# cindytsai/multigrid_poisson_solver

Hardware: AMD Instinct MI355X
Metric: vcycle_mlups (higher is better)
Workload: dtype f64; 1 GPU; V(3,3)-cycle N=8192^2 fp64, 11 levels to N=8, red-black GS(1e-7) coarse solve, cycle-file driver (eager, stream smoother: temporally blocked wave-streaming kernels on the large levels, register-tile kernels on the levels 65..1024, one-workgroup LDS kernel below; halos recomputed, neighbours via DPP lane shifts); N=8192, levels=11

## Files before the change

multigrid_poisson_solver_amd/csrc/mg_cycle.cpp:

```cpp
#include <chrono>
#include <cmath>
#include <cstdarg>
#include <cstdlib>
#include <cstring>
#include <algorithm>
#include <fstream>
#include <map>
#include <sstream>
#include <string>
#include <vector>

#include "mg_internal.h"

namespace mg {
namespace {

struct LevelNode {
    int N = 0;
    double *U = nullptr, *F = nullptr, *D = nullptr;
    LevelNode *nextNode = nullptr, *prevNode = nullptr;
    int step = 0;
    double smoothingError = 0.0;
    int pending_pre = 0;
    int descents = 0;
};

class LevelList {
public:
    explicit LevelList(Pool *pool, size_t elem_bytes = sizeof(double)) : pool_(pool), elem_bytes_(elem_bytes) {}
    ~LevelList() { clear(); }
    void clear()
    {
        while (lastNode_) Remove_back();
        init_ = 1;
    }
    void Push_back(int n)
    {
        LevelNode *nd = new LevelNode;
        const size_t bytes = (size_t)n * n * elem_bytes_;
        nd->N = n;
        nd->U = (double *)pool_->get(bytes);
        nd->F = (double *)pool_->get(bytes);
        nd->D = (double *)pool_->get(bytes);
        if (!firstNode_) {
            firstNode_ = lastNode_ = nd;
            return;
        }
        nd->prevNode = lastNode_;
        lastNode_->nextNode = nd;
        lastNode_ = nd;
    }
    void Remove_back()
    {
        LevelNode *nd = lastNode_;
        if (!nd) return;
        pool_->put(nd->U);
        pool_->put(nd->F);
        pool_->put(nd->D);
        if (firstNode_ == lastNode_) {
            firstNode_ = lastNode_ = nullptr;
        } else {
            lastNode_ = nd->prevNode;
            lastNode_->nextNode = nullptr;
            if (firstNode_ == lastNode_) init_ = 0;
        }
        delete nd;
    }
    LevelNode *last() { return lastNode_; }
    LevelNode *first() { return firstNode_; }
    int depth() const
    {
        int d = 0;
        for (LevelNode *p = firstNode_; p; p = p->nextNode) ++d;
        return d;
    }
    int Get_N() const { return lastNode_->N; }
    int Get_prev_N() const { return lastNode_->prevNode->N; }
    int Get_init() const { return init_; }
    void Set_init(int r) { init_ = r; }
    bool Is_firstNode() const { return firstNode_ == lastNode_ && firstNode_ != nullptr; }

private:
    Pool *pool_;
    size_t elem_bytes_;
    LevelNode *firstNode_ = nullptr, *lastNode_ = nullptr;
    int init_ = 1;
};

struct Text {
    std::string s;
    void printf(const char *fmt, ...)
    {
        char tmp[256];
        va_list ap;
        va_start(ap, fmt);
        vsnprintf(tmp, sizeof tmp, fmt, ap);
        va_end(ap);
        s += tmp;
    }
};

struct ReportItem {
    std::string text;
    int record = -1;
};

}
}

using namespace mg;

struct mg_cycle_plan {
    int flags = 0;
    std::string path;
    double L = 1.0, min_x = 0.0, min_y = 0.0;
    int con_step = 0, con_N = 0, N_max = 0, N_min = 0;
    std::vector<int> sizes;
    std::vector<double> tokens;
    Pool pool;
    LevelList *levels = nullptr;
    double *F_finest = nullptr;
    double *F64 = nullptr, *U64 = nullptr;
    int refinements = 1;
    int refine_it = 0;
    float *F32_res = nullptr;
    bool F32_stale = false;
    double *refine_err_dev = nullptr;
    std::vector<double> refine_err;
    double *err_dev = nullptr;
    size_t err_cap = 0;
    std::vector<mg_node_record> records;
    std::vector<ReportItem> report_items;
    std::string report;
    double *final_U = nullptr;
    int final_N = 0;
    hipGraph_t graph = nullptr;
    hipGraphExec_t graph_exec = nullptr;
    bool graph_ready = false, graph_failed = false;
    int warm_runs = 0;
    hipEvent_t ev_start = nullptr, ev_end[2] = {nullptr, nullptr};
    int end_at = 0;
    bool have_end = false;
    hipStream_t end_stream = nullptr;
    hipEvent_t mark0 = nullptr, mark1 = nullptr;
    NormSink norms;
    std::vector<Context::PendingNorm> graph_norms;
    int last_status = 0;
    bool last_replayed = false;
    std::vector<NodeOp> ops;
    std::vector<k::TailArgs> tails;
    struct Group {
        int depth = 0, first = 0;
        std::vector<int> members;
        size_t items_at = 0;
        std::vector<double *> errs;
    };
    std::vector<Group> sched;
    void *sched_items = nullptr;
    bool sched_ready = false, sched_tried = false;
    int sched_max_batch = 0;
    int sched_smoother = 0;
    double *sched_U = nullptr;
    int sched_N = 0;
    int *gs_slots = nullptr;
    int last_tail = -1;
};

namespace mg {
k::TailArgsF tail_args_f32(const k::TailArgs &a)
{
    k::TailArgsF f;
    memset(&f, 0, sizeof f);
    f.n_levels = a.n_levels;
    f.n_nodes = a.n_nodes;
    for (int i = 0; i < a.n_nodes; ++i) f.nodes[i] = a.nodes[i];
    for (int l = 0; l < a.n_levels; ++l) {
        f.N[l] = a.N[l];
        f.dx2[l] = (float)a.dx2[l];
        f.inv[l] = (float)a.inv[l];
        f.gs_h2[l] = a.gs_h2[l];
        f.gs_inv[l] = a.gs_inv[l];
        if (l + 1 < a.n_levels) {
            const RestrictTable &rt = restrict_table(a.N[l], a.N[l + 1]);
            const ProlongTable &pt = prolong_table(a.N[l + 1], a.N[l]);
            f.r_lo[l] = rt.lo;
            f.r_w[l] = rt.w_f;
            f.p_orow[l] = pt.owner_row;
            f.p_ocol[l] = pt.owner_col;
            f.p_rhi[l] = pt.row_hi_f;
            f.p_rlo[l] = pt.row_lo_f;
            f.p_chi[l] = pt.col_hi_f;
            f.p_clo[l] = pt.col_lo_f;
            f.c_dx[l] = (float)pt.c_dx;
        }
    }
    f.err_dev = a.err_dev;
    f.gs_state = a.gs_state;
    f.trace = a.trace;
    return f;
}

bool scan_tail(const std::vector<double> &tokens, size_t *tok_io, const std::vector<int> &sizes, int at0, int con_step,
               int top_N, double L, k::TailArgs *out, int *node_level)
{
    static const bool disabled = getenv("MG_NO_TAIL") != nullptr;
    if (disabled || con_step < 1 || top_N > k::TAIL_MAX_N || top_N < 3) return false;
    k::TailArgs &a = *out;
    memset(&a, 0, sizeof a);
    a.N[0] = top_N;
    int depth = 0, max_depth = 0, at = at0, n_nodes = 0;
    size_t tok = *tok_io;
    for (;;) {
        if (tok >= tokens.size()) return false;
        const int node = (int)tokens[tok++];
        if (node == 1 && depth == 0) {
            --tok;
            break;
        }
        if (n_nodes >= k::TAIL_MAX_NODES) return false;
        k::TailNode nd;
        memset(&nd, 0, sizeof nd);
        nd.type = node;
        nd.err_slot = -1;
        if (node == -1) {
            if (at + 1 >= (int)sizes.size() || depth + 1 >= k::TAIL_MAX_LEVELS) return false;
            nd.steps = con_step;
            node_level[n_nodes] = depth;
            ++depth;
            a.N[depth] = sizes[(size_t)++at];
            if (a.N[depth] < 3) return false;
            if (depth > max_depth) max_depth = depth;
        } else if (node == 0) {
            if (tok + 1 >= tokens.size()) return false;
            nd.tol = tokens[tok++];
            if ((int)tokens[tok++] != 1) return false;
            node_level[n_nodes] = depth;
        } else if (node == 1) {
            nd.steps = con_step;
            --depth;
            --at;
            node_level[n_nodes] = depth;
        } else {
            return false;
        }
        a.nodes[n_nodes++] = nd;
    }
    if (n_nodes == 0 || at != at0) return false;
    a.n_nodes = n_nodes;
    a.n_levels = max_depth + 1;
    if (!k::tail_fits(a)) return false;
    for (int l = 0; l < a.n_levels; ++l) {
        const double dx = L / (double)(a.N[l] - 1);
        a.dx2[l] = dx * dx;
        a.inv[l] = 1.0 / a.dx2[l];
        a.gs_h2[l] = a.dx2[l];
        a.gs_inv[l] = a.inv[l];
        if (l + 1 < a.n_levels) {
            const RestrictTable &rt = restrict_table(a.N[l], a.N[l + 1]);
            const ProlongTable &pt = prolong_table(a.N[l + 1], a.N[l]);
            if (!rt.lo || !pt.owner_row) return false;
            a.r_lo[l] = rt.lo;
            a.r_w[l] = rt.w;
            a.p_orow[l] = pt.owner_row;
            a.p_ocol[l] = pt.owner_col;
            a.p_rhi[l] = pt.row_hi;
            a.p_rlo[l] = pt.row_lo;
            a.p_chi[l] = pt.col_hi;
            a.p_clo[l] = pt.col_lo;
            a.c_dx[l] = pt.c_dx;
        }
    }
    *tok_io = tok;
    return true;
}
}

namespace {

const double TRIGGER = 0.01;

struct Exec {
    mg_cycle_plan *p;
    Context &c;
    size_t tok = 0;
    int at = 0;
    int status = 0;
    bool capturing = false;
    bool widened = false;
    bool tracing = false;
    bool untraceable = false;

    bool next(double *v)
    {
        if (tok >= p->tokens.size()) return false;
        *v = p->tokens[tok++];
        return true;
    }
    bool next_int(int *v)
    {
        double d;
        if (!next(&d)) return false;
        *v = (int)d;
        return true;
    }
};

int add_record(mg_cycle_plan *p, int node, int N, int steps)
{
    mg_node_record r{node, N, steps, 0.0};
    p->records.push_back(r);
    return (int)p->records.size() - 1;
}

void report_text(mg_cycle_plan *p, const char *t)
{
    if (!(p->flags & MG_CYCLE_REPORT)) return;
    ReportItem it;
    it.text = t;
    p->report_items.push_back(it);
}
void report_smoothing(mg_cycle_plan *p, int record)
{
    if (!(p->flags & MG_CYCLE_REPORT)) return;
    ReportItem it;
    it.record = record;
    p->report_items.push_back(it);
}

double *error_slot(mg_cycle_plan *p, int record) { return p->err_dev + record; }

int trigger_smoothing(Exec &x, LevelNode *lv)
{
    double slope = TRIGGER + 1.0, before = 0.0;
    lv->step = 0;
    while (slope > TRIGGER) {
        mg_doSmoothing(lv->N, x.p->L, lv->U, lv->F, 1, &lv->smoothingError);
        if (x.c.last_error) return lv->step;
        lv->step += 1;
        if (lv->step == 1) {
            before = lv->smoothingError;
            continue;
        }
        slope = std::fabs(lv->smoothingError - before);
        before = lv->smoothingError;
    }
    return lv->step;
}

int matching_up_step(const Exec &x)
{
    const mg_cycle_plan *p = x.p;
    if (p->con_step > 0) return p->con_step;
    if (p->con_step != 0) return -1;
    int depth = 1;
    for (size_t tok = x.tok; tok < p->tokens.size();) {
        const int node = (int)p->tokens[tok++];
        if (node == 2) break;
        if (node == -1) {
            if (tok >= p->tokens.size()) break;
            const int s = (int)p->tokens[tok++];
            if (p->con_N == 0) ++tok;
            if (s != 0) ++depth;
        } else if (node == 0) {
            tok += 2;
        } else if (node == 1) {
            if (tok >= p->tokens.size()) break;
            const int s = (int)p->tokens[tok++];
            if (--depth == 0) return s;
        }
    }
    return -1;
}

void ensure_U(mg_cycle_plan *p, LevelNode *lv)
{
    if (!lv || lv->pending_pre <= 0) return;
    if (p->flags & MG_CYCLE_MIXED) return;
    mg_smooth_pp(lv->N, p->L, nullptr, lv->U, lv->F, lv->pending_pre, nullptr, nullptr, -1);
    lv->pending_pre = 0;
}

void smooth_level(Exec &x, LevelNode *lv, int step, bool zero_start, bool want_D, int record)
{
    mg_cycle_plan *p = x.p;
    const size_t n = (size_t)lv->N * lv->N;
    if (p->flags & MG_CYCLE_FUSED) {
        if (zero_start) {
            mg_smooth_pp(lv->N, p->L, nullptr, lv->U, lv->F, step, error_slot(p, record), want_D ? lv->D : nullptr, -1);
        } else if (!want_D) {
            mg_smooth_pp(lv->N, p->L, lv->U, lv->D, lv->F, step, error_slot(p, record), nullptr, -1);
            std::swap(lv->U, lv->D);
        } else {
            double *tmp = (double *)p->pool.get(n * sizeof(double));
            mg_smooth_pp(lv->N, p->L, lv->U, tmp, lv->F, step, error_slot(p, record), lv->D, -1);
            std::swap(lv->U, tmp);
            p->pool.put(tmp);
        }
        return;
    }
    if (zero_start) mg_fill_zero(lv->U, n);
    {
        double *tmp = (double *)p->pool.get(n * sizeof(double));
        mg_smooth_pp(lv->N, p->L, lv->U, tmp, lv->F, step, error_slot(p, record), nullptr, +1);
        mg_copy(lv->U, tmp, n);
        p->pool.put(tmp);
    }
    if (want_D) {
        mg_getResidual(lv->N, p->L, lv->U, lv->F, lv->D);
        mg_negate(lv->N, lv->D);
    }
}

bool try_tail(Exec &x)
{
    mg_cycle_plan *p = x.p;
    LevelList &cycle = *p->levels;
    if (p->con_N != 1) return false;
    LevelNode *top = cycle.last();
    static const int batch_tail_n = [] { const char *e = getenv("MG_BATCH_TAIL_N"); return e ? atoi(e) : 32; }();
    if (x.tracing && top->N > batch_tail_n) return false;

    k::TailArgs a;
    int node_level[k::TAIL_MAX_NODES];
    size_t tok = x.tok;
    if (!scan_tail(p->tokens, &tok, p->sizes, x.at, p->con_step, top->N, p->L, &a, node_level)) return false;
    const int n_nodes = a.n_nodes;
    if (p->records.size() + (size_t)n_nodes > p->err_cap) return false;
    const int rec0 = (int)p->records.size();
    const char *down = "             *\n             |\n Restriction |\n             |\n             *\n";
    const char *up = "             *\n             |\nProlongation |\n             |\n             *\n";
    for (int i = 0; i < n_nodes; ++i) {
        k::TailNode &nd = a.nodes[i];
        const int N = a.N[node_level[i]];
        if (nd.type == -1) {
            const int rec = add_record(p, -1, N, nd.steps);
            nd.err_slot = rec - rec0;
            report_smoothing(p, rec);
            report_text(p, down);
        } else if (nd.type == 0) {
            add_record(p, 0, N, 0);
            if (p->flags & MG_CYCLE_REPORT) {
                Text t;
                t.printf("          ~Exact Solver~\n");
                t.printf("Current Grid Size N = %d\n", N);
                t.printf("   Use Exact Solver = GaussSeidel Even / Odd\n");
                t.printf("       Target Error = %.3e\n", nd.tol);
                report_text(p, t.s.c_str());
            }
        } else {
            const int rec = add_record(p, 1, N, nd.steps);
            nd.err_slot = rec - rec0;
            report_text(p, up);
            report_smoothing(p, rec);
        }
    }
    if (p->flags & MG_CYCLE_MIXED) {
        k::TailArgsF f = tail_args_f32(a);
        f.F_top = (const float *)top->F;
        f.U_top = (float *)top->U;
        f.err_dev = p->err_dev + rec0;
        f.gs_state = x.c.gs_state;
        ProfScope ps("coarse_tail_f32", top->N, 0.0);
        k::tail_launch_f32(x.c.stream, f);
        x.tok = tok;
        return true;
    }
    a.F_top = top->F;
    a.U_top = top->U;
    a.err_dev = p->err_dev + rec0;
    a.gs_state = x.c.gs_state;
    if (x.tracing) {
        NodeOp op;
        op.kind = 2;
        op.node.N = top->N;
        op.node.F = top->F;
        op.node.out = top->U;
        op.tail = (int)p->tails.size();
        p->tails.push_back(a);
        p->ops.push_back(op);
        x.tok = tok;
        return true;
    }
    static const bool trace_on = getenv("MG_TAIL_TRACE") != nullptr;
    static int traced = 0;
    long long *trace = nullptr;
    if (trace_on && traced < 3 && !x.capturing) {
        (void)hipMalloc((void **)&trace, (k::TAIL_MAX_NODES + 2 + 24 * 8) * sizeof(long long));
        (void)hipMemset(trace, 0, (k::TAIL_MAX_NODES + 2 + 24 * 8) * sizeof(long long));
        a.trace = trace;
    }
    {
        ProfScope ps("coarse_tail", top->N, 0.0);
        k::tail_launch(x.c.stream, a);
    }
    if (trace) {
        std::vector<long long> t((size_t)a.n_nodes + 2);
        (void)hipStreamSynchronize(x.c.stream);
        (void)hipMemcpy(t.data(), trace, t.size() * sizeof(long long), hipMemcpyDeviceToHost);
        ++traced;
        fprintf(stderr, "[tail trace] staging %.2f us;", (double)(t[1] - t[0]) * 0.01);
        for (int i = 0; i < a.n_nodes; ++i)
            fprintf(stderr, " %d@%d:%.2f", a.nodes[i].type, a.N[node_level[i]], (double)(t[(size_t)i + 2] - t[(size_t)i + 1]) * 0.01);
        fprintf(stderr, " us\n");
#ifdef MG_TAIL_PHASES
        std::vector<long long> ph(24 * 8);
        (void)hipMemcpy(ph.data(), trace + k::TAIL_MAX_NODES + 2, ph.size() * sizeof(long long), hipMemcpyDeviceToHost);
        for (int i = 0; i < a.n_nodes && i < 24; ++i) {
            if (a.nodes[i].type == 0) continue;
            fprintf(stderr, "[tail phases] %2d@%-3d cycles:", a.nodes[i].type, a.N[node_level[i]]);
            for (int k = 1; k < 8 && ph[(size_t)i * 8 + k]; ++k) fprintf(stderr, " %lld", ph[(size_t)i * 8 + k] - ph[(size_t)i * 8 + k - 1]);
            fprintf(stderr, "\n");
        }
#endif
        (void)hipFree(trace);
    }
    x.tok = tok;
    return true;
}

bool uses_trigger(const mg_cycle_plan *p);

void run_nodes(Exec &x)
{
    mg_cycle_plan *p = x.p;
    LevelList &cycle = *p->levels;
    const bool fused = (p->flags & MG_CYCLE_FUSED) != 0;
    const bool mixed = (p->flags & MG_CYCLE_MIXED) != 0;
    x.c.defer_norms = true;
    if (!x.tracing) {
        p->norms.begin_window();
        x.c.norm_sink = &p->norms;
    }
    auto fusable_down = [&](int N, int M, int step) {
        const RestrictTable &rt = restrict_table(N, M);
        return step >= 1 && step <= k::stream_max_steps() && x.c.smoother != SMOOTHER_SIMPLE && k::stream_fusable(N) && rt.lo && rt.fusable;
    };
    auto fusable_up = [&](int Nc, int N, int step) {
        const ProlongTable &pt = prolong_table(Nc, N);
        return step >= 1 && step <= k::stream_max_steps() && x.c.smoother != SMOOTHER_SIMPLE && k::stream_fusable(N) && pt.owner_row && pt.fusable;
    };

    for (;;) {
        int node;
        if (!x.next_int(&node)) break;
        if (node == 2) break;
        if (x.c.last_error) { x.status = 10; break; }
        if (p->records.size() >= p->err_cap) { x.status = 11; break; }

        if (node == -1) {
            int step = 0, next_N = 0;
            if (p->con_step == 0) { if (!x.next_int(&step)) { x.status = 3; break; } }
            else step = p->con_step;
            if (p->con_N == 0) { if (!x.next_int(&next_N)) { x.status = 3; break; } }
            else {
                if (x.at + 1 >= (int)p->sizes.size()) { x.status = 4; break; }
                next_N = p->sizes[++x.at];
            }
            if (step == 0) continue;
            if (next_N < 3) { x.status = 7; break; }
            if (x.tracing && (step < 1 || !fused || mixed)) { x.untraceable = true; break; }

            LevelNode *lv = cycle.last();
            const bool keep = (cycle.Get_init() == 0 && cycle.Is_firstNode());
            int rec;
            if (step == -1) {
                if (x.capturing) { x.status = 8; break; }
                if (!keep) mg_fill_zero(lv->U, (size_t)lv->N * lv->N);
                const int done = trigger_smoothing(x, lv);
                rec = add_record(p, -1, lv->N, done);
                p->records[rec].error = lv->smoothingError;
                mg_upload(error_slot(p, rec), &lv->smoothingError, 1);
                mg_getResidual(lv->N, p->L, lv->U, lv->F, lv->D);
                mg_negate(lv->N, lv->D);
                report_smoothing(p, rec);
                cycle.Push_back(next_N);
                if (!cycle.last()->U || !cycle.last()->F || !cycle.last()->D) { x.status = 14; break; }
                mg_restrict_signed(lv->N, lv->D, next_N, cycle.last()->F, +1);
            } else if (mixed) {
                if (keep) { x.status = 15; break; }
                rec = add_record(p, -1, lv->N, step);
                report_smoothing(p, rec);
                cycle.Push_back(next_N);
                if (!cycle.last()->U || !cycle.last()->F || !cycle.last()->D) { x.status = 14; break; }
                lv->pending_pre = 0;
                if (p->con_step > 0 && recompute_available(next_N, lv->N, step, p->con_step)) {
                    smooth_restrict_f32_no_out(lv->N, p->L, (float *)lv->U, (float *)lv->F, step, error_slot(p, rec), next_N,
                                               (float *)cycle.last()->F);
                    lv->pending_pre = step;
                } else {
                    mg_smooth_restrict_f32(lv->N, p->L, nullptr, (float *)lv->U, (float *)lv->F, step, error_slot(p, rec), next_N,
                                           (float *)cycle.last()->F);
                }
                if (x.c.last_error) { x.status = 15; break; }
                report_text(p, "             *\n             |\n Restriction |\n             |\n             *\n");
                if (!try_tail(x) && next_N <= k::TAIL_MAX_N) { x.status = 15; break; }
                continue;
            } else if (fused) {
                if (x.tracing) {
                    if (keep || !fusable_down(lv->N, next_N, step)) { x.untraceable = true; break; }
                    if (lv->descents > 0) {
                        const size_t bytes = (size_t)lv->N * lv->N * sizeof(double);
                        p->pool.put(lv->U);
                        p->pool.put(lv->D);
                        lv->U = (double *)p->pool.get(bytes);
                        lv->D = (double *)p->pool.get(bytes);
                        lv->pending_pre = 0;
                    }
                }
                lv->descents++;
                rec = add_record(p, -1, lv->N, step);
                report_smoothing(p, rec);
                cycle.Push_back(next_N);
                if (!cycle.last()->U || !cycle.last()->F || !cycle.last()->D || !lv->U || !lv->D) { x.status = 14; break; }
                double *Fc = cycle.last()->F;
                lv->pending_pre = 0;
                const int up_step = keep ? -1 : matching_up_step(x);
                if (up_step > 0 && recompute_available(next_N, lv->N, step, up_step)) {
                    smooth_restrict_no_out(lv->N, p->L, lv->U, lv->F, step, error_slot(p, rec), next_N, Fc);
                    lv->pending_pre = step;
                } else if (!keep) {
                    mg_smooth_restrict(lv->N, p->L, nullptr, lv->U, lv->F, step, error_slot(p, rec), next_N, Fc);
                } else {
                    double *tmp = (double *)p->pool.get((size_t)lv->N * lv->N * sizeof(double));
                    mg_smooth_restrict(lv->N, p->L, lv->U, tmp, lv->F, step, error_slot(p, rec), next_N, Fc);
                    std::swap(lv->U, tmp);
                    p->pool.put(tmp);
                }
                report_text(p, "             *\n             |\n Restriction |\n             |\n             *\n");
                try_tail(x);
                continue;
            } else {
                rec = add_record(p, -1, lv->N, step);
                smooth_level(x, lv, step, !keep, true, rec);
                report_smoothing(p, rec);
                cycle.Push_back(next_N);
                if (!cycle.last()->U || !cycle.last()->F || !cycle.last()->D) { x.status = 14; break; }
                mg_restrict_signed(lv->N, lv->D, next_N, cycle.last()->F, +1);
            }
            report_text(p, "             *\n             |\n Restriction |\n             |\n             *\n");
        } else if (node == 0) {
            double tol;
            int option;
            if (!x.next(&tol) || !x.next_int(&option)) { x.status = 3; break; }
            LevelNode *lv = cycle.last();
            if (x.tracing) { x.untraceable = true; break; }
            if (mixed) { x.status = 15; break; }
            if (x.capturing && lv->N > k::gs_single_workgroup_max_n()) { x.status = 8; break; }
            mg_doExactSolver(lv->N, p->L, lv->U, lv->F, tol, option);
            if (x.c.last_error) { x.status = 5; break; }
            add_record(p, 0, lv->N, 0);
            if (p->flags & MG_CYCLE_REPORT) {
                Text t;
                t.printf("          ~Exact Solver~\n");
                t.printf("Current Grid Size N = %d\n", lv->N);
                if (option == 0) t.printf("   Use Exact Solver = Inverse Matrix\n");
                if (option == 1) t.printf("   Use Exact Solver = GaussSeidel Even / Odd\n");
                t.printf("       Target Error = %.3e\n", tol);
                report_text(p, t.s.c_str());
            }
        } else if (node == 1) {
            int step;
            if (p->con_step == 0) { if (!x.next_int(&step)) { x.status = 3; break; } }
            else step = p->con_step;
            if (p->con_N != 0) x.at--;
            if (cycle.depth() < 2) { x.status = 6; break; }

            LevelNode *coarse = cycle.last();
            LevelNode *fine = coarse->prevNode;
            const char *arrow = "             *\n             |\nProlongation |\n             |\n             *\n";
            if (mixed) {
                if (step <= 0) { x.status = 15; break; }
                const int rec = add_record(p, 1, fine->N, step);
                const bool last_node = fine->N == p->N_max && p->refine_it == 0 && k::stream_fusable(fine->N) &&
                                       prolong_table(coarse->N, fine->N).fusable &&
                                       (x.tok >= p->tokens.size() || (int)p->tokens[x.tok] == 2);
                const int pre = fine->pending_pre;
                if (pre > 0 && !recompute_available(coarse->N, fine->N, pre, step)) { x.status = 15; break; }
                fine->pending_pre = 0;
                if (last_node) {
                    if (pre > 0)
                        prolong_smooth_f32_recompute(coarse->N, (const float *)coarse->U, fine->N, p->L, nullptr, p->U64, (const float *)fine->F,
                                                     pre, step, error_slot(p, rec));
                    else
                        prolong_smooth_f32_wide(coarse->N, (const float *)coarse->U, fine->N, p->L, (const float *)fine->U, p->U64,
                                                (const float *)fine->F, step, error_slot(p, rec));
                    x.widened = true;
                } else if (pre > 0) {
                    prolong_smooth_f32_recompute(coarse->N, (const float *)coarse->U, fine->N, p->L, (float *)fine->U, nullptr,
                                                 (const float *)fine->F, pre, step, error_slot(p, rec));
                } else {
                    mg_prolong_smooth_f32(coarse->N, (const float *)coarse->U, fine->N, p->L, (const float *)fine->U, (float *)fine->D,
                                          (float *)fine->F, step, error_slot(p, rec));
                    std::swap(fine->U, fine->D);
                }
                if (x.c.last_error) { x.status = 15; break; }
                cycle.Remove_back();
                report_text(p, arrow);
                report_smoothing(p, rec);
                continue;
            }
            if (x.tracing && (coarse->pending_pre > 0 || !fused || !fusable_up(coarse->N, fine->N, step) ||
                              (fine->pending_pre > 0 && !recompute_available(coarse->N, fine->N, fine->pending_pre, step)))) {
                x.untraceable = true;
                break;
            }
            ensure_U(p, coarse);
            if (fused && step > 0 && fine->pending_pre > 0 && recompute_available(coarse->N, fine->N, fine->pending_pre, step)) {
                const int rec = add_record(p, 1, fine->N, step);
                prolong_smooth_recompute(coarse->N, coarse->U, fine->N, p->L, fine->U, fine->F, fine->pending_pre, step, error_slot(p, rec));
                fine->pending_pre = 0;
                cycle.Remove_back();
                report_text(p, arrow);
                report_smoothing(p, rec);
                continue;
            }
            ensure_U(p, fine);
            if (fused && step > 0) {
                const int rec = add_record(p, 1, fine->N, step);
                mg_prolong_smooth(coarse->N, coarse->U, fine->N, p->L, fine->U, fine->D, fine->F, step,
                                  error_slot(p, rec));
                std::swap(fine->U, fine->D);
                cycle.Remove_back();
                report_text(p, arrow);
                report_smoothing(p, rec);
                continue;
            }
            if (fused) {
                mg_prolongAdd(coarse->N, coarse->U, fine->N, fine->U, fine->D);
                std::swap(fine->U, fine->D);
                cycle.Remove_back();
            } else {
                const size_t nf = (size_t)fine->N * fine->N;
                double *tempU = (double *)p->pool.get(nf * sizeof(double));
                mg_doProlongation(coarse->N, coarse->U, fine->N, tempU);
                cycle.Remove_back();
                mg_doGridAddition(fine->N, fine->U, tempU);
                p->pool.put(tempU);
            }
            report_text(p, arrow);

            if (step == 0) continue;
            LevelNode *lv = cycle.last();
            int rec;
            if (step == -1) {
                if (x.capturing) { x.status = 8; break; }
                const int done = trigger_smoothing(x, lv);
                rec = add_record(p, 1, lv->N, done);
                p->records[rec].error = lv->smoothingError;
                mg_upload(error_slot(p, rec), &lv->smoothingError, 1);
            } else {
                rec = add_record(p, 1, lv->N, step);
                smooth_level(x, lv, step, false, false, rec);
            }
            report_smoothing(p, rec);
        }
    }
    if (x.status == 0 && cycle.last() && cycle.last()->pending_pre > 0) {
        if (x.tracing) x.untraceable = true;
        else if (mixed) x.status = 15;
        else ensure_U(p, cycle.last());
    }
    x.c.norm_sink = nullptr;
    if (!x.tracing && uses_trigger(p)) p->norms.finish(x.c.stream);
    x.c.defer_norms = false;
}

void reset_levels(mg_cycle_plan *p)
{
    LevelList &cycle = *p->levels;
    while (cycle.depth() > 1) cycle.Remove_back();
    cycle.Set_init(1);
    if (cycle.first()) cycle.first()->descents = 0;
    p->records.clear();
    p->report_items.clear();
}

bool same_shape(const mg_cycle_plan *p, const NodeOp &a, const NodeOp &b)
{
    if (a.kind != b.kind || a.node.N != b.node.N) return false;
    if (a.kind == 2) {
        const k::TailArgs &x = p->tails[(size_t)a.tail], &y = p->tails[(size_t)b.tail];
        if (x.n_levels != y.n_levels || x.n_nodes != y.n_nodes) return false;
        for (int l = 0; l < x.n_levels; ++l)
            if (x.N[l] != y.N[l]) return false;
        for (int i = 0; i < x.n_nodes; ++i) {
            const k::TailNode &m = x.nodes[i], &n = y.nodes[i];
            if (m.type != n.type || m.steps != n.steps || m.err_slot != n.err_slot || m.tol != n.tol) return false;
        }
        return true;
    }
    const k::SmoothNode<double> &x = a.node, &y = b.node;
    return x.steps == y.steps && x.pre == y.pre && x.no_out == y.no_out && x.d_sign == y.d_sign && (x.in == nullptr) == (y.in == nullptr) &&
           (x.coarse == nullptr) == (y.coarse == nullptr) && (x.Fc == nullptr) == (y.Fc == nullptr) && x.Nc == y.Nc && x.M == y.M && a.L == b.L;
}

void drop_schedule(mg_cycle_plan *p)
{
    p->sched.clear();
    p->ops.clear();
    p->tails.clear();
    p->sched_ready = false;
    if (p->sched_items) (void)hipFree(p->sched_items);
    p->sched_items = nullptr;
    if (p->gs_slots) p->pool.put(p->gs_slots);
    p->gs_slots = nullptr;
    p->last_tail = -1;
    p->pool.park(false);
    p->pool.release_parked();
}

void build_schedule(mg_cycle_plan *p)
{
    static const bool on = [] { const char *e = getenv("MG_CYCLE_BATCH"); return !e || atoi(e) != 0; }();
    p->sched_tried = true;
    const bool mixed = (p->flags & MG_CYCLE_MIXED) != 0, fused = (p->flags & MG_CYCLE_FUSED) != 0;
    if (!on || !fused || mixed || p->con_N != 1 || p->con_step < 1 || getenv("MG_NO_TAIL")) return;
    {
        std::vector<int> descents(1, 0);
        bool points = false;
        for (size_t tok = 0; tok < p->tokens.size() && !points;) {
            const int node = (int)p->tokens[tok++];
            if (node == 2) break;
            if (node == -1) {
                if (descents.back() > 0) points = true;
                descents.back()++;
                descents.push_back(0);
            } else if (node == 0) {
                tok += 2;
            } else if (node == 1) {
                if (descents.size() < 2) break;
                descents.pop_back();
            }
        }
        if (!points) return;
    }
    Context &c = ctx();
    reset_levels(p);
    c.active_pool = &p->pool;
    p->pool.park(true);
    c.trace = &p->ops;
    c.trace_failed = false;
    static const int batch_recompute_min = [] { const char *e = getenv("MG_BATCH_RECOMPUTE_MIN_N"); return e ? atoi(e) : 1024; }();
    if (!getenv("MG_RECOMPUTE_MIN_N")) c.recompute_min_override = batch_recompute_min;
    Exec x{p, c};
    x.tracing = true;
    run_nodes(x);
    c.recompute_min_override = 0;
    c.trace = nullptr;
    c.active_pool = nullptr;
    const bool ok = x.status == 0 && !x.untraceable && !c.trace_failed && !c.last_error && !p->ops.empty();
    c.trace_failed = false;
    if (!ok) {
        drop_schedule(p);
        return;
    }
    std::map<const void *, int> wrote, read;
    auto depth_of = [](const std::map<const void *, int> &m, const void *k) {
        const auto it = m.find(k);
        return it == m.end() ? 0 : it->second;
    };
    std::vector<int> depth(p->ops.size(), 0);
    for (size_t i = 0; i < p->ops.size(); ++i) {
        const NodeOp &op = p->ops[i];
        const k::SmoothNode<double> &o = op.node;
        const void *in[3] = {o.F, (op.kind != 2 && o.pre == 0) ? (const void *)o.in : nullptr, o.coarse};
        const void *out[2] = {(op.kind == 2 || !o.no_out) ? (const void *)o.out : nullptr, o.Fc};
        int d = 0;
        for (const void *q : in)
            if (q) d = std::max(d, depth_of(wrote, q));
        for (const void *q : out)
            if (q) d = std::max(d, std::max(depth_of(wrote, q), depth_of(read, q)));
        depth[i] = ++d;
        for (const void *q : in)
            if (q) read[q] = std::max(depth_of(read, q), d);
        for (const void *q : out)
            if (q) wrote[q] = d;
    }
    for (size_t i = 0; i < p->ops.size(); ++i) {
        mg_cycle_plan::Group *g = nullptr;
        for (auto &cand : p->sched)
            if (cand.depth == depth[i] && same_shape(p, p->ops[(size_t)cand.first], p->ops[i])) { g = &cand; break; }
        if (!g) {
            p->sched.emplace_back();
            g = &p->sched.back();
            g->depth = depth[i];
            g->first = (int)i;
        }
        g->members.push_back((int)i);
    }
    std::stable_sort(p->sched.begin(), p->sched.end(), [](const mg_cycle_plan::Group &a, const mg_cycle_plan::Group &b) {
        return a.depth != b.depth ? a.depth < b.depth : a.first < b.first;
    });
    p->sched_max_batch = 0;
    for (const auto &g : p->sched) p->sched_max_batch = std::max(p->sched_max_batch, (int)g.members.size());
    if (p->sched_max_batch < 2) {
        drop_schedule(p);
        return;
    }
    if (!p->tails.empty()) {
        p->gs_slots = (int *)p->pool.get(2 * p->tails.size() * sizeof(int));
        if (!p->gs_slots) { drop_schedule(p); return; }
        for (size_t t = 0; t < p->tails.size(); ++t) p->tails[t].gs_state = p->gs_slots + 2 * t;
    }
    std::vector<char> host;
    for (auto &g : p->sched) {
        g.items_at = host.size();
        for (int m : g.members) {
            const NodeOp &o = p->ops[(size_t)m];
            if (o.kind == 2) {
                const k::TailArgs &a = p->tails[(size_t)o.tail];
                const TailBatchItem it{a.F_top, a.U_top, a.err_dev, a.gs_state};
                host.insert(host.end(), (const char *)&it, (const char *)&it + sizeof it);
                p->last_tail = std::max(p->last_tail, o.tail);
            } else {
                const NodeBatchItem it{o.node.in, o.node.F, o.node.coarse, o.node.out, o.node.Fc};
                host.insert(host.end(), (const char *)&it, (const char *)&it + sizeof it);
                g.errs.push_back(o.node.err);
            }
        }
        while (host.size() % 16) host.push_back(0);
    }
    if (hipMalloc(&p->sched_items, host.size()) != hipSuccess || hipMemcpy(p->sched_items, host.data(), host.size(), hipMemcpyHostToDevice) != hipSuccess) {
        (void)hipGetLastError();
        drop_schedule(p);
        return;
    }
    p->pool.park(false);
    p->sched_U = p->final_U = p->levels->last()->U;
    p->sched_N = p->final_N = p->levels->last()->N;
    p->sched_smoother = (int)c.smoother;
    p->sched_ready = true;
    if (getenv("MG_CYCLE_DEBUG")) {
        fprintf(stderr, "[cycle] batched schedule: %zu nodes in %zu launches (largest batch %d), %.1f MiB of arrays\n", p->ops.size(), p->sched.size(),
                p->sched_max_batch, (double)p->pool.bytes_held() / 1048576.0);
        for (const auto &g : p->sched)
            fprintf(stderr, "   depth %2d  %-44s N=%5d x%zu\n", g.depth, p->ops[(size_t)g.first].kind == 2 ? "coarse_tail" : p->ops[(size_t)g.first].name,
                    p->ops[(size_t)g.first].node.N, g.members.size());
    }
}

void replay_schedule(mg_cycle_plan *p)
{
    Context &c = ctx();
    c.defer_norms = true;
    c.norms_at_window_end = true;
    p->norms.begin_window();
    c.norm_sink = &p->norms;
    for (const auto &g : p->sched) {
        const NodeOp &o = p->ops[(size_t)g.first];
        const int n = (int)g.members.size();
        if (o.kind == 2) {
            ProfScope ps(n > 1 ? "coarse_tail (batch)" : "coarse_tail", o.node.N, 0.0);
            k::tail_launch(c.stream, p->tails[(size_t)o.tail], n, (const TailBatchItem *)((const char *)p->sched_items + g.items_at));
        } else if (n == 1) {
            replay_node(o, nullptr);
        } else {
            NodeBatch b;
            b.n = n;
            b.dev = (const NodeBatchItem *)((const char *)p->sched_items + g.items_at);
            b.err_outs = g.errs.data();
            replay_node(o, &b);
        }
    }
    c.norm_sink = nullptr;
    c.defer_norms = false;
    c.norms_at_window_end = false;
    if (p->last_tail >= 0)
        (void)hipMemcpyAsync(c.gs_state, p->gs_slots + 2 * p->last_tail, 2 * sizeof(int), hipMemcpyDeviceToDevice, c.stream);
}

bool uses_trigger(const mg_cycle_plan *p)
{
    if (p->con_step == -1) return true;
    if (p->con_step != 0) return false;
    for (double t : p->tokens)
        if (t == -1.0) return true;
    return false;
}

}

extern "C" {

mg_cycle_plan *mg_cycle_load(const char *path, int flags)
{
    if (!require_ready("mg_cycle_load")) return nullptr;
    std::ifstream f(path);
    if (!f.is_open()) {
        fail(MG_ERR_CYCLE_FILE, "Cannot open file %s", path);
        return nullptr;
    }
    mg_cycle_plan *p = new mg_cycle_plan;
    p->pool.poison(pool_poison_wanted());
    p->norms.pool = &p->pool;
    p->flags = flags;
    p->path = path;
    if (!(f >> p->L >> p->min_x >> p->min_y >> p->con_step >> p->con_N >> p->N_max >> p->N_min)) {
        fail(MG_ERR_CYCLE_FILE, "%s: malformed cycle structure header", path);
        delete p;
        return nullptr;
    }
    if (p->N_max < 3 || p->N_max > 46340 || (p->con_N != 0 && p->N_min < 1)) {
        fail(MG_ERR_CYCLE_FILE, "%s: unusable grid sizes N_max=%d N_min=%d", path, p->N_max, p->N_min);
        delete p;
        return nullptr;
    }
    std::string tok;
    while (f >> tok) {
        char *end = nullptr;
        const double v = strtod(tok.c_str(), &end);
        if (end == tok.c_str()) break;
        p->tokens.push_back(v);
    }
    if (p->con_N == 1) {
        for (int n = p->N_max; n >= p->N_min && n > 0; n /= 2) p->sizes.push_back(n);
    } else if (p->con_N == 2) {
        for (int n = p->N_max; n >= p->N_min; --n) p->sizes.push_back(n);
    }
    size_t nodes = 0;
    for (double t : p->tokens)
        if (t == -1.0 || t == 1.0 || t == 0.0) ++nodes;
    p->err_cap = nodes + 8;
    p->err_dev = (double *)p->pool.get(p->err_cap * sizeof(double));
    const bool mixed = (flags & MG_CYCLE_MIXED) != 0;
    if (mixed && (!(flags & MG_CYCLE_FUSED) || p->con_N != 1 || p->con_step < 1 || p->con_step > k::stream_max_steps())) {
        fail(MG_ERR_UNSUPPORTED, "%s: the mixed-precision mode needs the fused driver, con_N = 1 and a fixed con_step in 1..%d",
             path, k::stream_max_steps());
        delete p;
        return nullptr;
    }
    p->levels = new LevelList(&p->pool, mixed ? sizeof(float) : sizeof(double));
    p->levels->Push_back(p->N_max);
    LevelNode *top = p->levels->last();
    if (!top->U || !top->F || !top->D || !p->err_dev) {
        mg_cycle_destroy(p);
        return nullptr;
    }
    if (mixed) {
        const size_t n = (size_t)top->N * top->N;
        p->F64 = (double *)p->pool.get(n * sizeof(double));
        p->U64 = (double *)p->pool.get(n * sizeof(double));
        if (!p->F64 || !p->U64) {
            mg_cycle_destroy(p);
            return nullptr;
        }
        mg_getSource(top->N, p->L, p->F64, p->min_x, p->min_y);
        mg_to_f32((float *)top->F, p->F64, n);
    } else {
        mg_getSource(top->N, p->L, top->F, p->min_x, p->min_y);
    }
    p->F_finest = top->F;
    static const bool fenced = [] { const char *e = getenv("MG_WINDOW_EVENT_FENCE"); return e && atoi(e) != 0; }();
    for (hipEvent_t *e : {&p->ev_start, &p->ev_end[0], &p->ev_end[1]}) (void)hipEventCreateWithFlags(e, fenced ? hipEventDefault : hipEventDisableSystemFence);
    mg_sync();
    return p;
}

int mg_cycle_enqueue(mg_cycle_plan *p)
{
    if (!require_ready("mg_cycle_enqueue") || !p) return 1;
    Context &c = ctx();
    hipStream_t s = c.stream;
    int status = 0;
    if (!p->sched_tried) build_schedule(p);
    const bool want_graph = (p->flags & MG_CYCLE_GRAPH) && (p->flags & MG_CYCLE_FUSED) && !(p->flags & MG_CYCLE_MIXED) &&
                            !uses_trigger(p) && !p->graph_failed && (!p->sched_ready || (int)c.smoother == p->sched_smoother);
    c.profile_window++;
    const bool timed = !stream_is_capturing(s);
    p->mark0 = p->mark1 = nullptr;
    if (timed) {
        hipEvent_t prev = (p->have_end && p->end_stream == s) ? p->ev_end[p->end_at] : nullptr;
        const hipError_t q = prev ? hipEventQuery(prev) : hipSuccess;
        if (q != hipSuccess) (void)hipGetLastError();
        if (prev && q == hipErrorNotReady) {
            p->mark0 = prev;
        } else {
            (void)hipEventRecord(p->ev_start, s);
            p->mark0 = p->ev_start;
        }
    }

    p->last_replayed = false;
    if (want_graph && p->graph_ready) {
        if (!MG_HIP(hipGraphLaunch(p->graph_exec, s))) status = 9;
        p->last_replayed = status == 0;
        p->norms.pending = p->graph_norms;
        p->norms.unfinished = true;
    } else {
        const bool mixed = (p->flags & MG_CYCLE_MIXED) != 0;
        const int outer = mixed ? p->refinements : 1;
        const size_t n_top = (size_t)p->N_max * p->N_max;
        if (mixed && p->F32_stale) {
            k::convert_to_f32(s, (float *)p->levels->first()->F, p->F64, n_top);
            p->F32_stale = false;
        }
        const bool use_sched = p->sched_ready && (int)c.smoother == p->sched_smoother;
        if (use_sched) {
            p->final_U = p->sched_U;
            p->final_N = p->sched_N;
            const bool capture_now = want_graph && p->warm_runs >= 1;
            bool capturing = false;
            if (capture_now) {
                if (hipStreamBeginCapture(s, hipStreamCaptureModeThreadLocal) == hipSuccess) capturing = true;
                else { (void)hipGetLastError(); p->graph_failed = true; }
            }
            replay_schedule(p);
            status = c.last_error ? 10 : 0;
            if (capturing) {
                hipGraph_t g = nullptr;
                const hipError_t e = hipStreamEndCapture(s, &g);
                if (e == hipSuccess && status == 0 && hipGraphInstantiate(&p->graph_exec, g, nullptr, nullptr, 0) == hipSuccess) {
                    p->graph = g;
                    p->graph_ready = true;
                    p->graph_norms = p->norms.pending;
                    if (!MG_HIP(hipGraphLaunch(p->graph_exec, s))) status = 9;
                    p->last_replayed = status == 0;
                } else {
                    (void)hipGetLastError();
                    if (g) (void)hipGraphDestroy(g);
                    p->graph_failed = true;
                    replay_schedule(p);
                    status = c.last_error ? 10 : 0;
                }
            }
            p->warm_runs++;
        }
        for (int it = 0; it < outer && status == 0 && !use_sched; ++it) {
        reset_levels(p);
        c.active_pool = &p->pool;
        p->refine_it = it;
        if (it > 0) {
            const double dx = p->L / (double)(p->N_max - 1);
            float *dst = p->F32_res ? p->F32_res : (float *)p->levels->first()->F;
            k::refine_residual(s, p->N_max, 1.0 / (dx * dx), p->U64, p->F64, dst, p->refine_err_dev + (it - 1));
            if (p->F32_res) p->levels->first()->F = (double *)p->F32_res;
            else p->F32_stale = true;
        }
        Exec x{p, c};
        const bool capture_now = want_graph && p->warm_runs >= 1;
        if (capture_now) {
            if (hipStreamBeginCapture(s, hipStreamCaptureModeThreadLocal) == hipSuccess) x.capturing = true;
            else { (void)hipGetLastError(); p->graph_failed = true; }
        }
        static const bool dbg = getenv("MG_CYCLE_DEBUG") != nullptr;
        if (dbg) fprintf(stderr, "[cycle] run_nodes: capturing=%d\n", (int)x.capturing);
        run_nodes(x);
        status = x.status;
        if (dbg) fprintf(stderr, "[cycle] run_nodes done: status %d\n", status);
        if (x.capturing) {
            hipGraph_t g = nullptr;
            const hipError_t e = hipStreamEndCapture(s, &g);
            if (dbg) fprintf(stderr, "[cycle] end capture: %s\n", hipGetErrorString(e));
            if (e == hipSuccess && status == 0 && hipGraphInstantiate(&p->graph_exec, g, nullptr, nullptr, 0) == hipSuccess) {
                if (dbg) fprintf(stderr, "[cycle] instantiated\n");
                p->graph = g;
                p->graph_ready = true;
                p->graph_norms = p->norms.pending;
                if (!MG_HIP(hipGraphLaunch(p->graph_exec, s))) status = 9;
                p->last_replayed = status == 0;
                if (dbg) fprintf(stderr, "[cycle] launched: status %d\n", status);
            } else {
                (void)hipGetLastError();
                if (g) (void)hipGraphDestroy(g);
                p->graph_failed = true;
                if (status == 8) status = 0;
                reset_levels(p);
                Exec y{p, c};
                run_nodes(y);
                status = y.status;
            }
        }
        c.active_pool = nullptr;
        p->warm_runs++;
        p->levels->first()->F = p->F_finest;
        LevelNode *last = p->levels->last();
        p->final_U = last->U;
        p->final_N = last->N;
        if (mixed && status == 0 && last->N == p->N_max) {
            if (x.widened) {  }
            else if (it == 0) k::convert_to_f64(s, p->U64, (const float *)last->U, n_top);
            else k::add_widened(s, p->U64, (const float *)last->U, n_top);
            p->final_U = p->U64;
        } else if (mixed && status == 0) {
            status = 15;
        }
        }
    }
    if (timed) {
        p->end_at ^= 1;
        (void)hipEventRecord(p->ev_end[p->end_at], s);
        p->mark1 = p->ev_end[p->end_at];
        p->have_end = true;
        p->end_stream = s;
    }
    p->last_status = status;
    return status;
}

int mg_cycle_collect(mg_cycle_plan *p, mg_cycle_result *out)
{
    if (!require_ready("mg_cycle_collect") || !p) return 1;
    Context &c = ctx();
    memset(out, 0, sizeof *out);
    p->norms.finish(c.stream);
    mg_sync();
    float dev_ms = 0.f;
    if (p->mark0 && p->mark1 && hipEventElapsedTime(&dev_ms, p->mark0, p->mark1) != hipSuccess) (void)hipGetLastError();

    if (!p->records.empty()) {
        std::vector<double> all(p->records.size());
        mg_download(all.data(), p->err_dev, all.size());
        for (size_t i = 0; i < p->records.size(); ++i)
            if (p->records[i].node != 0) p->records[i].error = all[i];
    }

    p->refine_err.clear();
    if ((p->flags & MG_CYCLE_MIXED) && p->refinements > 1 && p->refine_err_dev) {
        p->refine_err.resize((size_t)p->refinements - 1);
        mg_download(p->refine_err.data(), p->refine_err_dev, p->refine_err.size());
    }

    double mg_error = 0.0;
    if (p->flags & (MG_CYCLE_ERROR | MG_CYCLE_REPORT))
        mg_analyticError(p->final_N, p->L, p->final_U, p->min_x, p->min_y, &mg_error);

    if (p->flags & MG_CYCLE_REPORT) {
        Text t;
        for (const ReportItem &it : p->report_items) {
            if (it.record < 0) {
                t.s += it.text;
                continue;
            }
            const mg_node_record &r = p->records[it.record];
            t.printf("          ~Smoothing~\n");
            t.printf("Current Grid Size N = %d\n", r.N);
            t.printf("    Smoothing Steps = %d\n", r.steps);
            t.printf("              Error = %lf\n", r.error);
        }
        t.printf("\n\n===== Final Result =====\n    Error = %lf\n", mg_error);
        p->report = t.s;
    }

    out->status = p->last_status ? p->last_status : (c.last_error ? 10 : 0);
    out->N = p->final_N;
    out->U_dev = p->final_U;
    out->mg_error = mg_error;
    out->time_ms = 0.0;
    out->device_ms = dev_ms;
    out->n_records = (int)p->records.size();
    out->records = p->records.data();
    out->report = p->report.c_str();
    out->graph_replayed = p->last_replayed ? 1 : 0;
    out->schedule_launches = (p->sched_ready && (int)c.smoother == p->sched_smoother) ? (int)p->sched.size() : 0;
    return out->status;
}

int mg_cycle_execute(mg_cycle_plan *p, mg_cycle_result *out)
{
    if (!require_ready("mg_cycle_execute") || !p) return 1;
    mg_sync();
    const auto t0 = std::chrono::steady_clock::now();
    mg_cycle_enqueue(p);
    mg_sync();
    const auto t1 = std::chrono::steady_clock::now();
    const int status = mg_cycle_collect(p, out);
    out->time_ms = std::chrono::duration<double, std::milli>(t1 - t0).count();
    return status;
}

int mg_cycle_set_refinement(mg_cycle_plan *p, int cycles)
{
    if (!require_ready("mg_cycle_set_refinement") || !p) return 1;
    if (!(p->flags & MG_CYCLE_MIXED) || cycles < 1 || cycles > 64) {
        fail(MG_ERR_ARG, "mg_cycle_set_refinement: needs a MG_CYCLE_MIXED plan and 1..64 cycles (got %d)", cycles);
        return 1;
    }
    if (!p->refine_err_dev) {
        p->refine_err_dev = (double *)p->pool.get(64 * sizeof(double));
        if (!p->refine_err_dev) return 1;
    }
    if (cycles > 1 && !p->F32_res) p->F32_res = (float *)p->pool.get((size_t)p->N_max * p->N_max * sizeof(float));
    p->refinements = cycles;
    return 0;
}

int mg_cycle_refinement_errors(mg_cycle_plan *p, double *out, int cap)
{
    if (!p || !out) return 0;
    int n = 0;
    for (; n < (int)p->refine_err.size() && n < cap; ++n) out[n] = p->refine_err[(size_t)n];
    return n;
}

void mg_cycle_destroy(mg_cycle_plan *p)
{
    if (!p) return;
    if (ctx().ready) (void)hipStreamSynchronize(ctx().stream);
    if (p->graph_exec) (void)hipGraphExecDestroy(p->graph_exec);
    if (p->graph) (void)hipGraphDestroy(p->graph);
    for (hipEvent_t e : {p->ev_start, p->ev_end[0], p->ev_end[1]})
        if (e) (void)hipEventDestroy(e);
    if (p->levels) {
        p->levels->clear();
        delete p->levels;
    }
    drop_schedule(p);
    p->norms.release();
    if (p->err_dev) p->pool.put(p->err_dev);
    if (p->refine_err_dev) p->pool.put(p->refine_err_dev);
    if (p->F32_res) p->pool.put(p->F32_res);
    if (p->F64) p->pool.put(p->F64);
    if (p->U64) p->pool.put(p->U64);
    p->pool.trim();
    delete p;
}

int mg_print2File(int N, const double *U_dev, const char *file_name)
{
    if (!require_ready("mg_print2File")) return 1;
    std::vector<double> U((size_t)N * N);
    mg_download(U.data(), U_dev, U.size());
    FILE *o = fopen(file_name, "w");
    if (!o) {
        fail(MG_ERR_ARG, "Cannot open file %s", file_name);
        return 1;
    }
    for (int j = N - 1; j >= 0; --j)
        for (int i = 0; i < N; ++i) fprintf(o, i == N - 1 ? "%lf\n" : "%lf,", U[i + (size_t)N * j]);
    fclose(o);
    return 0;
}

int mg_cycle_main(int argc, char **argv)
{
    if (argc != 3) {
        printf("[ ERROR ]: Wrong input numbers of parameter.\n");
        return 1;
    }
    printf("OpenMP threads = %d\n", atoi(argv[1]));
    printf("Cycle structure file name = %s\n", argv[2]);
    const char *dev = getenv("MG_DEVICE");
    if (mg_init(dev ? atoi(dev) : 0) != 0) return 1;
    const char *mixed = getenv("MG_MIXED"), *refine = getenv("MG_REFINE");
    const bool want_mixed = (mixed && atoi(mixed) != 0) || (refine && atoi(refine) > 1);
    mg_cycle_plan *plan = mg_cycle_load(argv[2], MG_CYCLE_FUSED | MG_CYCLE_REPORT | MG_CYCLE_ERROR | (want_mixed ? MG_CYCLE_MIXED : 0));
    if (!plan) {
        printf("[ ERROR ]: Cannot open file %s\n", argv[2]);
        return 1;
    }
    if (refine && atoi(refine) > 1 && mg_cycle_set_refinement(plan, atoi(refine)) != 0) {
        printf("[ ERROR ]: %s\n", mg_last_error_string());
        mg_cycle_destroy(plan);
        return 1;
    }
    mg_cycle_result res;
    if (const char *w = getenv("MG_WARMUP"))
        for (int i = 0; i < atoi(w); ++i) mg_cycle_execute(plan, &res);
    const int status = mg_cycle_execute(plan, &res);
    if (status != 0) {
        printf("[ ERROR ]: cycle structure file is malformed (status %d)\n", status);
        mg_cycle_destroy(plan);
        return 1;
    }
    fputs(res.report, stdout);
    printf("Time Used = %lf (ms)\n", res.time_ms);
    std::string name = std::string("Sol_HIP_") + argv[2];
    mg_print2File(res.N, res.U_dev, name.c_str());
    printf("Output file name = %s\n", name.c_str());
    mg_cycle_destroy(plan);
    mg_finalize();
    return 0;
}

}
```

multigrid_poisson_solver_amd/csrc/mg_internal.h:

```cpp
#pragma once

#include <hip/hip_runtime_api.h>

#include <cstddef>
#include <cstdint>
#include <cstdio>
#include <map>
#include <string>
#include <utility>
#include <vector>

#include "mg_hip.h"

namespace mg {

enum ErrorCode {
    MG_OK = 0,
    MG_ERR_HIP = 1,
    MG_ERR_ARG = 2,
    MG_ERR_UNSUPPORTED = 3,
    MG_ERR_NOT_INIT = 4,
    MG_ERR_CYCLE_FILE = 5,
    MG_ERR_COMM = 6,
};

void fail(int code, const char *fmt, ...);
bool hip_ok(hipError_t e, const char *what, const char *file, int line);
#define MG_HIP(expr) ::mg::hip_ok((expr), #expr, __FILE__, __LINE__)

struct RestrictTable {
    int *lo = nullptr;
    double *w = nullptr;
    int *inv = nullptr;
    double *inv_w = nullptr;
    float *w_f = nullptr, *inv_w_f = nullptr;
    bool fusable = false;
};
struct ProlongTable {
    int *owner_row = nullptr, *owner_col = nullptr;
    double *row_hi = nullptr, *row_lo = nullptr;
    double *col_hi = nullptr, *col_lo = nullptr;
    float *row_hi_f = nullptr, *row_lo_f = nullptr, *col_hi_f = nullptr, *col_lo_f = nullptr;
    double c_dx = 0.0;
    bool fusable = false;
    bool fusable4 = false;
    bool closed_form = false;
};
inline const double *weights_as(double, const double *w, const float *) { return w; }
inline const float *weights_as(float, const double *, const float *w_f) { return w_f; }

struct RowWindow {
    int base = 0, rows = 0, own_lo = 0, own_hi = 0;
    int norm_lo = -1, norm_hi = -1;
};

class Pool {
public:
    void *get(size_t bytes);
    void put(void *p);
    void trim();
    size_t bytes_held() const { return held_; }
    void park(bool on) { park_ = on; }
    void release_parked();
    void poison(bool on) { poison_ = on; }
private:
    std::multimap<size_t, void *> free_;
    std::map<void *, size_t> live_;
    std::vector<std::pair<size_t, void *>> parked_;
    bool park_ = false;
    bool poison_ = false;
    size_t held_ = 0;
};
bool pool_poison_wanted();
void poison_block(void *p, size_t bytes);

enum Smoother { SMOOTHER_STREAM = 0, SMOOTHER_SIMPLE = 1, SMOOTHER_STREAM_ONLY = 2 };

struct NodeOp;
struct NormSink;

struct Context {
    bool ready = false;
    int device = -1;
    hipStream_t own_stream = nullptr;
    hipStream_t stream = nullptr;
    int n_cu = 256;
    Pool pool;
    Pool *active_pool = nullptr;
    int recompute_min_override = 0;
    std::vector<NodeOp> *trace = nullptr;
    bool trace_failed = false;
    Smoother smoother = SMOOTHER_STREAM;
    int source_mode = 0;
    int source_identical = -1;
    double *partials = nullptr;
    size_t partials_cap = 0;
    std::vector<void *> retired;
    struct PendingNorm { const double *part; int n; int N; double *out; };
    bool defer_norms = false;
    bool norms_at_window_end = false;
    std::vector<PendingNorm> pending_norms;
    double *norm_arena = nullptr;
    size_t norm_arena_cap = 0, norm_arena_used = 0;
    size_t norm_window_total = 0;
    NormSink *norm_sink = nullptr;
    double *scalars = nullptr;
    int *gs_state = nullptr;
    double *host_scalars = nullptr;
    int *host_ints = nullptr;
    std::map<std::pair<int, int>, RestrictTable> rtab;
    std::map<std::pair<int, int>, ProlongTable> ptab;
    int last_error = 0;
    std::string last_error_text;
    bool abort_on_error = true;
    bool profiling = false;
    int profile_min_N = 0;
    int profile_every = 1;
    long profile_window = 0;
    struct ProfRec { std::string name; int N; double bytes; hipEvent_t e0, e1; };
    std::vector<ProfRec> prof;
    std::vector<hipEvent_t> event_pool;
    bool geometry_log = false;
    bool geometry_dropped = false;
    std::vector<int> geometry;
};

struct ProfScope {
    ProfScope(const char *name, int N, double algo_bytes, hipStream_t stream = nullptr);
    ~ProfScope();
    int slot = -1;
    hipStream_t on = nullptr;
};

Context &ctx();
void stream_geometry_record(const int (&rec)[MG_STREAM_GEOMETRY_FIELDS]);
bool require_ready(const char *who);
double *partials(size_t n);
Pool &scratch_pool();
double *norm_partials(size_t n);
void norm_finish(hipStream_t s, const double *part, size_t n, int N, double *out);
void flush_norms();
bool stream_is_capturing(hipStream_t s);

struct NormSink {
    struct Block { double *p; size_t cap; };
    Pool *pool = nullptr;
    std::vector<Block> blocks;
    size_t block = 0, used = 0;
    std::vector<Context::PendingNorm> pending;
    bool unfinished = false;
    void begin_window();
    double *take(size_t n);
    void flush(hipStream_t s);
    void finish(hipStream_t s);
    void release();
};

const RestrictTable &restrict_table(int N, int M);
const ProlongTable &prolong_table(int N, int M);
void build_restriction_table(int N, int M, int *lo, double *w);
void build_prolongation_table(int N, int M, int axis, int *owner, double *w_hi, double *w_lo);
void build_cubic_table(int N_src, int N_dst, int *base, double *w);
bool restriction_table_in_bounds(int N, int M, const int *lo);

void fill_source_rows(int N, double L, double min_x, double min_y, int row_lo, int row_hi, double *dev_dst);
struct SlabFusion {
    const double *coarse = nullptr;
    int Nc = 0;
    double *Fc = nullptr;
    int M = 0;
    RowWindow fine_w, coarse_w, fc_w;
    int pre = 0;
    bool no_out = false;
    double *out_wide = nullptr;
};
template <typename T>
void slab_smooth(int N, double L, const T *U_in, T *U_out, const T *F, int step, double *raw_norm_out, const SlabFusion &sf);

bool comm_ready();
void comm_set_stream(hipStream_t s);
int comm_rank();
int comm_size();
void comm_group_begin();
void comm_group_end();
void comm_send(const void *buf, size_t bytes, int peer);
void comm_recv(void *buf, size_t bytes, int peer);
void comm_allgather(const double *send, double *recv, size_t count_per_rank);

void parallel_for(size_t n, void (*fn)(size_t, size_t, void *), void *arg, size_t serial_below = 4096);

struct NodeBatchItem {
    const void *in, *F, *coarse;
    void *out, *Fc;
};
struct NodeBatch {
    int n = 0;
    const NodeBatchItem *dev = nullptr;
    double *const *err_outs = nullptr;
};
struct TailBatchItem {
    const void *F_top;
    void *U_top;
    double *err_dev;
    int *gs_state;
};
namespace k {
template <typename T>
struct SmoothNode {
    int N = 0;
    T dx2 = 0, inv = 0;
    const T *in = nullptr;
    const T *F = nullptr;
    T *out = nullptr;
    int steps = 0;
    double *err = nullptr;
    T *D = nullptr;
    int d_sign = -1;
    const T *coarse = nullptr;
    int Nc = 0;
    const ProlongTable *pt = nullptr;
    T *Fc = nullptr;
    int M = 0;
    const RestrictTable *rt = nullptr;
    const RowWindow *fine_w = nullptr, *coarse_w = nullptr, *fc_w = nullptr;
    int pre = 0;
    bool no_out = false;
    double *out_wide = nullptr;
    const NodeBatch *batch = nullptr;
    double cw = 0.25;
    double dc = 4.0;
    bool shifted = false;
};
struct Shifted {
    bool on = false;
    double d = 4.0, q = 0.25;
};
}

struct NodeOp {
    int kind = 0;
    double L = 1.0;
    k::SmoothNode<double> node;
    int tail = -1;
    char name[48] = {0};
    double bytes = 0.0;
};

namespace k {
void jacobi_simple(hipStream_t s, int N, double dx2, const double *in, const double *F, double *out);
void residual(hipStream_t s, int N, double inv, const double *U, const double *F, double *D, int sign, const Shifted &sh = {});
void smoothing_error(hipStream_t s, int N, double inv, const double *U, const double *F, double *out);
void finish_smoothing_error(hipStream_t s, const double *part, size_t n, int N, double *out);
constexpr int MAX_NORMS_PER_FLUSH = 160;
struct NormBatch {
    const double *part[MAX_NORMS_PER_FLUSH];
    double *out[MAX_NORMS_PER_FLUSH];
    int n[MAX_NORMS_PER_FLUSH];
    int N[MAX_NORMS_PER_FLUSH];
};
void finish_smoothing_errors(hipStream_t s, const NormBatch &b, int count);
int  stream_max_steps();
bool stream_supported(int N);
bool stream_fusable(int N);
bool stream_recompute_supported(int pre, int steps);
void jacobi_stream(hipStream_t s, const SmoothNode<double> &node);
bool tile_wanted(int N);
bool tile_wanted_slab(int N);
int  tile_max_steps();
void jacobi_tile(hipStream_t s, const SmoothNode<double> &node);
void jacobi_tile_f32(hipStream_t s, const SmoothNode<float> &node);
void restrict_gather(hipStream_t s, int N, const double *Uf, int M, double *Uc, const RestrictTable &t, int sign);
void prolong(hipStream_t s, int N, const double *Uc, int M, const double *Uf_in, double *Uf_out, const ProlongTable &t);
void restrict_gather_f32(hipStream_t s, int N, const float *Uf, int M, float *Uc, const RestrictTable &t, int sign);
void prolong_add_f32(hipStream_t s, int N, const float *Uc, int M, const float *Uf_in, float *Uf_out, const ProlongTable &t);
void convert_to_f32(hipStream_t s, float *dst, const double *src, size_t n);
void convert_to_f64(hipStream_t s, double *dst, const float *src, size_t n);
void refine_residual(hipStream_t s, int N, double inv, const double *U, const double *F, float *src, double *err_out);
void add_widened(hipStream_t s, double *U, const float *e, size_t n);
void refine_residual_rows(hipStream_t s, int N, double inv, const double *U, const double *F, float *src, const RowWindow &w,
                          double *out_raw);
void add(hipStream_t s, size_t n, double *a, const double *b);
void negate(hipStream_t s, size_t n, double *a);
void source_device(hipStream_t s, int N, double L, double *F, double min_x, double min_y, int row_lo, int row_hi);
void analytic(hipStream_t s, int N, double L, double *U, double min_x, double min_y);
void analytic_error(hipStream_t s, int N, double L, const double *U, double min_x, double min_y, double *out);
void analytic_error_rows(hipStream_t s, int N, double L, const double *U, const RowWindow &w, double min_x,
                         double min_y, double *out_raw);
void fill_uniform(hipStream_t s, double *dst, size_t n, uint64_t seed);
void checksum(hipStream_t s, const double *src, size_t n, uint64_t *out_dev );
void jacobi_stream_f32(hipStream_t s, const SmoothNode<float> &node);
constexpr int TAIL_MAX_LEVELS = 6;
constexpr int TAIL_MAX_NODES = 48;
constexpr int TAIL_MAX_N = 64;
struct TailNode {
    int type;
    int steps;
    int err_slot;
    int pad;
    double tol;
};
template <typename T>
struct TailArgsT {
    int n_levels, n_nodes;
    int N[TAIL_MAX_LEVELS];
    T dx2[TAIL_MAX_LEVELS], inv[TAIL_MAX_LEVELS];
    double gs_h2[TAIL_MAX_LEVELS], gs_inv[TAIL_MAX_LEVELS];
    const int *r_lo[TAIL_MAX_LEVELS];
    const T *r_w[TAIL_MAX_LEVELS];
    const int *p_orow[TAIL_MAX_LEVELS], *p_ocol[TAIL_MAX_LEVELS];
    const T *p_rhi[TAIL_MAX_LEVELS], *p_rlo[TAIL_MAX_LEVELS], *p_chi[TAIL_MAX_LEVELS], *p_clo[TAIL_MAX_LEVELS];
    T c_dx[TAIL_MAX_LEVELS];
    int tab_real0, tab_int0;
    long long *trace;
    const T *F_top;
    T *U_top;
    double *err_dev;
    int *gs_state;
    const TailBatchItem *batch;
    TailNode nodes[TAIL_MAX_NODES];
};
typedef TailArgsT<double> TailArgs;
typedef TailArgsT<float> TailArgsF;
void tail_launch_f32(hipStream_t s, const TailArgsF &a);
bool tail_fits(const TailArgs &a);
void tail_launch(hipStream_t s, const TailArgs &a, int n_batch = 1, const TailBatchItem *batch_dev = nullptr);
void gauss_seidel(hipStream_t s, int N, double h2, double inv, double *U, const double *F, double tol,
                  int *state);
void gauss_seidel_blocks_launch(hipStream_t s, int N, double h2, double inv, double *U, const double *F, double tol, int *state);
int  gs_single_workgroup_max_n();
void wjacobi(hipStream_t s, int N, double dx2, double cw, const double *in, const double *F, double *out, const Shifted &sh = {});
size_t resnorm_partials(int N);
void resnorm(hipStream_t s, int N, double inv, const double *U, const double *F, double *part, double *out, const Shifted &sh = {});
constexpr int GS_RELATIVE_MAX_N = 64;
bool gs_relative_fits(int N);
void gauss_seidel_relative(hipStream_t s, int N, double h2, double inv, double *U, const double *F, double atol, double rtol,
                           int max_iters, int *state, double *err_out, const Shifted &sh = {});
void resnorm_batch(hipStream_t s, int n, int N, double inv, bool has_u, const NodeBatchItem *items, double *part, double *out,
                   const Shifted &sh = {});
void gauss_seidel_relative_batch(hipStream_t s, int n, int N, double h2, double inv, const NodeBatchItem *items, double atol,
                                 double rtol, int max_iters, int *state, const Shifted &sh = {});
void residual_batch(hipStream_t s, int n, int N, double inv, const NodeBatchItem *items, int sign, const Shifted &sh = {});
void restrict_batch(hipStream_t s, int n, int N, int M, const NodeBatchItem *items, const RestrictTable &t, int sign);
void prolong_add_batch(hipStream_t s, int n, int N, int M, const NodeBatchItem *items, const ProlongTable &t);
void copy_batch(hipStream_t s, int n, size_t count, const NodeBatchItem *items);
struct CubicTable {
    int N_src = 0, N_dst = 0;
    int *base = nullptr;
    double *w = nullptr;
};
bool cubic_table_fits(int N_src, int N_dst, const int *base_host);
void prolong_cubic(hipStream_t s, const CubicTable &t, const double *Uc, double *Uf);
void rim_extract(hipStream_t s, int N, const double *U, double *g);
void rim_sample(hipStream_t s, const CubicTable &t, const double *g_f, double *g_c);
void rim_fill(hipStream_t s, int N, const double *g, double *U, bool zero_interior);
void flag_or(hipStream_t s, const int *gs_state, int *acc);
struct HeatConsts {
    double sigma = 0.0, beta = 0.0, gamma = 0.0, inv = 0.0;
    bool lap = false;
};
void heat_rhs(hipStream_t s, int N, const HeatConsts &c, const double *U, const double *Q, double *F);
void heat_rhs_batch(hipStream_t s, int n, int N, const HeatConsts &c, const NodeBatchItem *items);
void wjacobi_vc(hipStream_t s, int N, double dx2, double sd, double omega, const double *A, const double *in, const double *F,
                double *out);
void residual_vc(hipStream_t s, int N, double inv, double sd, const double *A, const double *U, const double *F, double *D, int sign);
void apply_vc(hipStream_t s, int N, double inv, double sd, const double *A, const double *U, double *out);
void resnorm_vc(hipStream_t s, int N, double inv, double sd, const double *A, const double *U, const double *F, double *part,
                double *out);
void gauss_seidel_relative_vc(hipStream_t s, int N, double h2, double inv, double sd, const double *A, double *U, const double *F,
                              double atol, double rtol, int max_iters, int *state, double *err_out);
void coef_coarsen(hipStream_t s, int N, const double *Af, int M, double *Ac, const RestrictTable &t);
void coef_check(hipStream_t s, const double *A, size_t n, int *flag);
void wjacobi_vc_batch(hipStream_t s, int n, int N, double dx2, double sd, double omega, bool zero_in, const NodeBatchItem *items);
void residual_vc_batch(hipStream_t s, int n, int N, double inv, double sd, const NodeBatchItem *items, int sign);
void resnorm_vc_batch(hipStream_t s, int n, int N, double inv, double sd, const NodeBatchItem *items, double *part, double *out);
void gauss_seidel_relative_vc_batch(hipStream_t s, int n, int N, double h2, double inv, double sd, const NodeBatchItem *items,
                                    double atol, double rtol, int max_iters, int *state);
void coef_coarsen_batch(hipStream_t s, int n, int N, int M, const NodeBatchItem *items, const RestrictTable &t);
void coef_check_batch(hipStream_t s, int n, size_t count, const NodeBatchItem *items, int *flags);
void heat_rhs_vc(hipStream_t s, int N, const HeatConsts &c, const double *A, const double *U, const double *Q, double *F);
void wjacobi_bc(hipStream_t s, int N, double dx2, double sd, double omega, const int *kind, const double *A, const double *in,
                const double *F, double *out);
void residual_bc(hipStream_t s, int N, double inv, double sd, const int *kind, const double *A, const double *U, const double *F,
                 double *D, int sign);
void apply_bc(hipStream_t s, int N, double inv, double sd, const int *kind, const double *A, const double *U, double *out);
void resnorm_bc(hipStream_t s, int N, double inv, double sd, const int *kind, const double *A, const double *U, const double *F,
                double *part, double *out);
void gauss_seidel_relative_bc(hipStream_t s, int N, double h2, double inv, double sd, const int *kind, const double *A, double *U,
                              const double *F, double atol, double rtol, int max_iters, int *state, double *err_out);
void gauss_seidel_relative_bc_mean(hipStream_t s, int N, double h2, double inv, const int *kind, const double *A, double *U,
                                   const double *F, double atol, double rtol, int max_iters, int *state, double *err_out,
                                   double *mean_out);
void weighted_mean(hipStream_t s, int N, const double *X, double target, double *part, double *out);
void shift_by(hipStream_t s, int N, const double *Xin, const double *c, double *Xout);
void restrict_bc(hipStream_t s, int N, const int *kind, const double *D, int M, double *Fc, const RestrictTable &t);
void prolong_add_bc(hipStream_t s, int M, const int *kind, const double *Uc, int N, const double *Uin, double *Uout, const int *lo,
                    const double *w);
void neumann_source(hipStream_t s, int N, double t, const int *kind, const double *A, const double *F, const double *G, double *Fout);
void heat_rhs_bc(hipStream_t s, int N, const HeatConsts &c, const int *kind, const double *A, const double *U, const double *Q,
                 double *F);
void wjacobi_rx(hipStream_t s, int N, double dx2, double sd, double omega, const double *A, const double *S, const double *in,
                const double *F, double *out);
void residual_rx(hipStream_t s, int N, double dx2, double inv, double sd, const double *A, const double *S, const double *U,
                 const double *F, double *D, int sign);
void apply_rx(hipStream_t s, int N, double dx2, double inv, double sd, const double *A, const double *S, const double *U, double *out);
void resnorm_rx(hipStream_t s, int N, double dx2, double inv, double sd, const double *A, const double *S, const double *U,
                const double *F, double *part, double *out);
void gauss_seidel_relative_rx(hipStream_t s, int N, double h2, double inv, double sd, const double *A, const double *S, double *U,
                              const double *F, double atol, double rtol, int max_iters, int *state, double *err_out);
void reaction_check(hipStream_t s, const double *S, size_t n, int *flag);
constexpr int KRYLOV_MAX_K = MG_KRYLOV_MAX_M - 1;
struct KrylovVecs {
    const double *q[KRYLOV_MAX_K];
    const double *z[KRYLOV_MAX_K];
};
size_t krylov_blocks(int N);
void krylov_dots(hipStream_t s, int N, int k, const double *q, const KrylovVecs &v, double *part, const double *w, double *b,
                 double *d_out);
void krylov_orth(hipStream_t s, int N, int k, double *q, double *z, const double *r, const KrylovVecs &v, const double *b,
                 double *part);
void krylov_orth_finish(hipStream_t s, int N, const double *part, int k, int m, double *gh, double *w_k, double *alpha, double *brk,
                        double *rec);
void krylov_update(hipStream_t s, int N, const double *alpha, double *U, const double *z, double *r, const double *q, double *part);
void krylov_update_finish(hipStream_t s, int N, const double *part, double *rr, double *rho_out, double *rec_tail);
void krylov_log_restart(hipStream_t s, double *rec_tail, const double *rho);
struct KrylovBatchItem {
    double *U, *r;
    double *zk, *qk;
    double *scal;
    double *part;
    double *rec;
    size_t off;
    int k, pad;
};
constexpr int KRYLOV_SCAL_B = 0, KRYLOV_SCAL_W = MG_KRYLOV_MAX_M, KRYLOV_SCAL_ALPHA = 2 * MG_KRYLOV_MAX_M,
              KRYLOV_SCAL_BRK = KRYLOV_SCAL_ALPHA + 1, KRYLOV_SCAL_COUNT = KRYLOV_SCAL_ALPHA + 2;
void krylov_zero_batch(hipStream_t s, int n, int N, const KrylovBatchItem *items);
void krylov_dots_batch(hipStream_t s, int n, int N, int kmax, const KrylovBatchItem *items, const KrylovVecs &v);
void krylov_orth_batch(hipStream_t s, int n, int N, int kmax, int m, const KrylovBatchItem *items, const KrylovVecs &v);
void krylov_update_batch(hipStream_t s, int n, int N, int m, const KrylovBatchItem *items, double *rb, int stride);
void krylov_log_restart_batch(hipStream_t s, int n, int m, const KrylovBatchItem *items, const double *norms);
void apply_vc_batch(hipStream_t s, int n, int N, double inv, double sd, const NodeBatchItem *items);
void coef_grad(hipStream_t s, int N, double h, const double *lam, const double *U, double *gA);
void rim_grad(hipStream_t s, int N, double inv, const double *A, const double *lam, const double *Ubar, double *gU);
void coef_grad_batch(hipStream_t s, int n, int N, double h, const NodeBatchItem *items);
void rim_grad_batch(hipStream_t s, int n, int N, double inv, const NodeBatchItem *items);
constexpr int EIGS_MAX_M = 3 * MG_EIGS_MAX_BLOCK;
constexpr int EIGS_TILE = 6;
inline int eigs_tiles(int m) { const int nt = (m + EIGS_TILE - 1) / EIGS_TILE; return nt * (nt + 1) / 2; }
constexpr int EIGS_TILE_SUMS = 2 * EIGS_TILE * EIGS_TILE;
size_t eigs_gram_blocks(int N);
size_t eigs_rotate_blocks(int N);
void eigs_gram(hipStream_t s, int N, int m, const double *const *ptrs, double *part, double *out);
constexpr int EIGS_COEF_CP = MG_EIGS_MAX_BLOCK * EIGS_MAX_M, EIGS_COEF_THETA = 2 * EIGS_COEF_CP,
              EIGS_COEF_COUNT = EIGS_COEF_THETA + MG_EIGS_MAX_BLOCK;
constexpr int EIGS_PTR_AS = EIGS_MAX_M, EIGS_PTR_R = 2 * EIGS_MAX_M, EIGS_PTR_COUNT = 2 * EIGS_MAX_M + MG_EIGS_MAX_BLOCK;
void eigs_rotate(hipStream_t s, int N, int m, int p, double *const *ptrs, const double *coef, double *part, double *res2);
void eigs_resnorm(hipStream_t s, int N, int p, double *const *ptrs, const double *coef, double *part, double *res2);
void eigs_start(hipStream_t s, int N, double *dst, const double *src);
}

bool solve_opts_ok(const char *who, int N, double L, const mg_solve_opts &o);
struct LevelConsts {
    double dx2, inv, sd, d, q, c;
    k::Shifted sh;
};
std::vector<LevelConsts> solve_level_consts(const std::vector<int> &sizes, double L, const mg_solve_opts &o);
struct SolveLevels {
    const std::vector<double *> *A, *B, *F;
    int *gs_state;
    double *gs_err;
};
struct SolveOperator {
    const mg_solve_opts *o;
    const std::vector<int> *sizes;
    const std::vector<LevelConsts> *lc;
    const int *kind = nullptr;
    const std::vector<double *> *coef = nullptr;
    const std::vector<int *> *p_lo = nullptr;
    const std::vector<double *> *p_w = nullptr;
    bool project_coarse = false;
    const std::vector<double *> *react = nullptr;

    const double *a(int l) const { return coef ? (*coef)[l] : nullptr; }
    const double *s(int l) const { return react ? (*react)[l] : nullptr; }
    void sweep(hipStream_t st, int l, const double *in, const double *F, double *out) const;
    void residual(hipStream_t st, int l, const double *U, const double *F, double *D) const;
    void restrict_residual(hipStream_t st, int l, const double *D, double *Fc) const;
    void coarse_solve(hipStream_t st, double *U, const double *F, int *gs_state, double *gs_err) const;
    void prolong_add(hipStream_t st, int l, const double *Uc, const double *Uin, double *Uout) const;
    void norm(hipStream_t st, const double *U, const double *F, double *part, double *out) const;
    void apply(hipStream_t st, const double *U, double *out) const;
};
enum class Field : int { None, U0, F0, A, B, F, Coef };
struct FieldRef {
    Field f = Field::None;
    int level = 0;
    bool operator==(const FieldRef &r) const { return f == r.f && level == r.level; }
};
struct SolveStep {
    enum Kind : int { Node, Sweep, Residual, Restrict, Coarse, ProlongAdd, Copy } kind;
    int level;
    int steps = 0, d_sign = 0;
    bool fused_transfer = false;
    FieldRef in, F, coarse, out, Fc;
    int slot = 0;
};
struct SolveCycle {
    std::vector<SolveStep> steps;
    int n_slots = 0;
};
SolveCycle build_solve_cycle(int nl, int pre, int post, int top, bool fused, const int *down_fused, const int *up_fused, bool with_coef);
void solve_fusable_levels(const std::vector<int> &sizes, std::vector<int> *down_fused, std::vector<int> *up_fused);
k::SmoothNode<double> solve_cycle_node(const SolveStep &s, const std::vector<int> &sizes, const std::vector<LevelConsts> &lc,
                                       const NodeBatchItem &it);
int run_solve_cycle(hipStream_t st, const SolveCycle &c, const SolveLevels &lv, const SolveOperator &op, const double *F0, double *U0);
const double *solver_coefficient(const mg_solver *s);
const int *solver_boundary(const mg_solver *s);
int solver_size(const mg_solver *s, double *L);
int batch_solver_size(const mg_batch_solver *s, double *L, int *max_batch);
const double *batch_solver_coefficient(const mg_batch_solver *s, int i);
int batch_solver_cycle(mg_batch_solver *s, hipStream_t st, int n, const double *const *F0, double *const *U0);
bool batch_solver_enqueue_state(mg_batch_solver *s, hipStream_t st);
bool batch_solver_coarse_capped(const mg_batch_solver *s, int n);

bool recompute_available(int Nc, int N, int pre, int step);
int  recompute_min_n();
void replay_node(const NodeOp &op, const NodeBatch *batch);
void smooth_restrict_no_out(int N, double L, double *U_unused, double *F, int step, double *error_dev, int M, double *F_c);
void prolong_smooth_recompute(int Nc, const double *U_c, int N, double L, double *U_out, double *F, int pre, int step, double *error_dev);
void smooth_restrict_f32_no_out(int N, double L, float *U_unused, float *F, int step, double *error_dev, int M, float *F_c);
void prolong_smooth_f32_recompute(int Nc, const float *U_c, int N, double L, float *U_out, double *U_out_wide, const float *F, int pre,
                                  int step, double *error_dev);
void prolong_smooth_f32_wide(int Nc, const float *U_c, int N, double L, const float *U_in, double *U_out_wide, const float *F,
                             int step, double *error_dev);
k::TailArgsF tail_args_f32(const k::TailArgs &a);
bool scan_tail(const std::vector<double> &tokens, size_t *tok_io, const std::vector<int> &sizes, int at0, int con_step,
               int top_N, double L, k::TailArgs *out, int *node_level);

}
```

multigrid_poisson_solver_amd/csrc/mg_tail.hip:

```cpp
#define MG_REAL double
#define MG_REAL_NS f64
#include "mg_tail_impl.h"

namespace mg {
namespace k {

__global__ __launch_bounds__(64) void k_gs_blocks(int N, double h2, double inv, double *U, const double *F, double tol, int *state)
{
    const int n = N * N, t = threadIdx.x;
    if (t < n) f64::lds[n + t] = F[t];
    __syncthreads();
    f64::gauss_seidel_blocks(N, h2, inv, 0, n, tol, state);
    if (t < n) U[t] = f64::lds[t];
}
void gauss_seidel_blocks_launch(hipStream_t s, int N, double h2, double inv, double *U, const double *F, double tol, int *state)
{
    hipLaunchKernelGGL(k_gs_blocks, dim3(1), dim3(64), (size_t)2 * N * N * sizeof(double), s, N, h2, inv, U, F, tol, state);
}

bool tail_fits(const TailArgs &a) { return f64::tail_lds_bytes(a) <= (size_t)(160 * 1024 - 512); }
void tail_launch(hipStream_t s, const TailArgs &a, int n_batch, const TailBatchItem *batch_dev) { f64::tail_launch(s, a, n_batch, batch_dev); }

}
}
```

multigrid_poisson_solver_amd/csrc/mg_tail_impl.h:

```cpp
#include <hip/hip_runtime.h>

#include <type_traits>

#include "mg_divconst.h"
#include "mg_gs_wave.h"
#include "mg_internal.h"

#if !defined(MG_REAL) || !defined(MG_REAL_NS)
#error "define MG_REAL (double|float) and MG_REAL_NS (f64|f32) before including mg_tail_impl.h"
#endif

namespace mg {
namespace k {
namespace MG_REAL_NS {

typedef MG_REAL real_t;


#ifndef MG_TAIL_THREADS
#define MG_TAIL_THREADS 1024
#endif
constexpr int TAIL_THREADS = MG_TAIL_THREADS;
constexpr int TAIL_WAVES = TAIL_THREADS / 64;

#define FOR_POINTS(N, r, c, p)                                             \
    for (int r = (int)(threadIdx.x >> 6); r < (N); r += TAIL_WAVES)        \
        for (int c = (int)(threadIdx.x & 63), p = r * (N) + c; c < (N); c += 64, p += 64)

__device__ __forceinline__ bool rim(int r, int c, int N) { return r == 0 || c == 0 || r == N - 1 || c == N - 1; }

__device__ __forceinline__ double wave_sum(double v)
{
#pragma unroll
    for (int o = 32; o > 0; o >>= 1) v += __shfl_down(v, o, 64);
    return v;
}
__device__ __forceinline__ double block_total(double v, double *sm )
{
    const int lane = threadIdx.x & 63, w = threadIdx.x >> 6;
    v = wave_sum(v);
    __syncthreads();
    if (lane == 0) sm[w] = v;
    __syncthreads();
    if (threadIdx.x == 0) {
        double r = 0.0;
        for (int i = 0; i < TAIL_THREADS / 64; ++i) r += sm[i];
        sm[16] = r;
    }
    __syncthreads();
    return sm[16];
}

extern __shared__ __align__(16) real_t lds[];
#define SRC(i) lds[src + (i)]
#define FF(i) lds[F + (i)]

constexpr int PT = (TAIL_MAX_N * TAIL_MAX_N + TAIL_THREADS - 1) / TAIL_THREADS;

template <int NP>
struct PointsT {
    int p[NP], r[NP], c[NP];
    bool live[NP], inner[NP], even[NP];
};
template <int NP>
__device__ __forceinline__ PointsT<NP> map_points(int N)
{
    PointsT<NP> P;
    const float rn = 1.0f / (float)N;
#pragma unroll
    for (int k = 0; k < NP; ++k) {
        const int p = (int)threadIdx.x + k * TAIL_THREADS;
        const int r = (int)(((float)p + 0.5f) * rn), c = p - r * N;
        P.p[k] = p;
        P.r[k] = r;
        P.c[k] = c;
        P.live[k] = p < N * N;
        P.inner[k] = P.live[k] && r > 0 && c > 0 && r < N - 1 && c < N - 1;
        P.even[k] = ((r + c) & 1) == 0;
    }
    return P;
}

template <bool ZERO, int NP>
__device__ __forceinline__ void sweep(const PointsT<NP> &P, int N, int src, int dst, real_t (&v)[NP], const real_t (&h2f)[NP])
{
#pragma unroll
    for (int k = 0; k < NP; ++k) {
        if (!P.live[k]) continue;
        const int p = P.p[k];
        real_t nv = v[k];
        if (P.inner[k]) {
            if (ZERO) {
                const real_t z = 0.0;
                nv = z + real_t(0.25) * (z + z + z + z - 4 * z - h2f[k]);
            } else {
                nv = v[k] + real_t(0.25) * (SRC(p + N) + SRC(p - N) + SRC(p + 1) + SRC(p - 1) - 4 * v[k] - h2f[k]);
            }
        }
        lds[dst + p] = nv;
        v[k] = nv;
    }
    __syncthreads();
}

__device__ __forceinline__ void post_partial(double acc, double *slots)
{
    const double t = gsw::wave_total(acc);
    if ((threadIdx.x & 63) == 0) slots[threadIdx.x >> 6] = t;
}
__device__ __forceinline__ void finish_error(const double *slots, int N, double *out)
{
    double s = 0.0;
#pragma unroll
    for (int i = 0; i < TAIL_WAVES; ++i) s += slots[i];
    double e = s + s;
    if ((N & (N - 1)) == 0) e = ldexp(e, -2 * (31 - __builtin_clz(N)));
    else e = e / N / N;
    *out = e;
}

#define GSD(o, i) (reinterpret_cast<double *>(lds)[(o) + (i)])

__device__ void gauss_seidel_block(int N, double h2, double inv, int u, int f, double tol, double *sm, int *state)
{
    FOR_POINTS(N, r, c, p) GSD(u, p) = 0.0;
    __syncthreads();
    const double denom = (double)((N - 2) * (N - 2));
    int iterations = 0;
    for (;;) {
        for (int colour = 0; colour < 2; ++colour) {
            FOR_POINTS(N, r, c, p)
            {
                if (!rim(r, c, N) && ((r + c) & 1) == colour)
                    GSD(u, p) = 0.25 * (GSD(u, p - 1) + GSD(u, p + 1) + GSD(u, p + N) + GSD(u, p - N) - h2 * GSD(f, p));
            }
            __syncthreads();
        }
        ++iterations;
        double acc = 0.0;
        FOR_POINTS(N, r, c, p)
        {
            if (!rim(r, c, N))
                acc = acc + fabs(inv * (GSD(u, p + N) + GSD(u, p - N) + GSD(u, p + 1) + GSD(u, p - 1) - 4 * GSD(u, p)) - GSD(f, p));
        }
        const double err = block_total(acc, sm) / denom;
        if (!(err > tol) || iterations >= 50000000) break;
    }
    if (threadIdx.x == 0) {
        state[0] = 1;
        state[1] = iterations;
    }
}

__device__ void gauss_seidel_level(int N, double h2, double inv, int src, int F, int scratch, double tol, double *sm, int *state)
{
    if (sizeof(real_t) == sizeof(double)) {
        gauss_seidel_block(N, h2, inv, src, F, tol, sm, state);
    } else {
        const int u = scratch, f = scratch + N * N;
        FOR_POINTS(N, r, c, p) GSD(f, p) = (double)FF(p);
        __syncthreads();
        gauss_seidel_block(N, h2, inv, u, f, tol, sm, state);
        __syncthreads();
        FOR_POINTS(N, r, c, p) SRC(p) = (real_t)GSD(u, p);
    }
}

constexpr int GS_WAVE_PTS = 4;
__device__ void gauss_seidel_wave_lds(int N, double h2, double inv, int u, bool in_place, int src, int F, double tol, int *state)
{
    if (threadIdx.x < 64) {
        const int lane = threadIdx.x, n = N * N;
        const float rn = 1.0f / (float)N;
        int q[GS_WAVE_PTS];
        bool live[GS_WAVE_PTS], inner[GS_WAVE_PTS], red[GS_WAVE_PTS];
        double f[GS_WAVE_PTS], h2f[GS_WAVE_PTS];
#pragma unroll
        for (int k = 0; k < GS_WAVE_PTS; ++k) {
            const int p = lane + 64 * k;
            const int r = (int)(((float)p + 0.5f) * rn), c = p - r * N;
            q[k] = p;
            live[k] = p < n;
            inner[k] = live[k] && r > 0 && c > 0 && r < N - 1 && c < N - 1;
            red[k] = ((r + c) & 1) == 0;
            f[k] = live[k] ? (double)FF(p) : 0.0;
            h2f[k] = h2 * f[k];
            if (live[k]) GSD(u, p) = 0.0;
        }
        const double denom = (double)((N - 2) * (N - 2));
        const double thr = tol * denom, thr_hi = thr * (1.0 + 0x1p-48), thr_lo = thr * (1.0 - 0x1p-48);
        double own[GS_WAVE_PTS], nw[GS_WAVE_PTS], ne[GS_WAVE_PTS], nn[GS_WAVE_PTS], ns[GS_WAVE_PTS];
#pragma unroll
        for (int k = 0; k < GS_WAVE_PTS; ++k) own[k] = nw[k] = ne[k] = nn[k] = ns[k] = 0.0;
        int iterations = 0;
        for (;;) {
#pragma unroll
            for (int k = 0; k < GS_WAVE_PTS; ++k) {
                if (inner[k] && red[k]) {
                    own[k] = 0.25 * (nw[k] + ne[k] + nn[k] + ns[k] - h2f[k]);
                    GSD(u, q[k]) = own[k];
                }
            }
#pragma unroll
            for (int k = 0; k < GS_WAVE_PTS; ++k) {
                if (inner[k] && !red[k]) {
                    const int p = q[k];
                    own[k] = 0.25 * (GSD(u, p - 1) + GSD(u, p + 1) + GSD(u, p + N) + GSD(u, p - N) - h2f[k]);
                    GSD(u, p) = own[k];
                }
            }
            ++iterations;
            double acc = 0.0;
#pragma unroll
            for (int k = 0; k < GS_WAVE_PTS; ++k) {
                if (inner[k]) {
                    const int p = q[k];
                    nw[k] = GSD(u, p - 1);
                    ne[k] = GSD(u, p + 1);
                    nn[k] = GSD(u, p + N);
                    ns[k] = GSD(u, p - N);
                    const double rs = inv * (nn[k] + ns[k] + ne[k] + nw[k] - 4 * own[k]) - f[k];
                    acc += fabs(rs);
                }
            }
            const double sum = gsw::wave_total(acc);
            const bool above = sum > thr_hi ? true : (sum < thr_lo ? false : sum / denom > tol);
            if (!above || iterations >= 50000000) break;
        }
        if (!in_place) {
#pragma unroll
            for (int k = 0; k < GS_WAVE_PTS; ++k)
                if (live[k]) SRC(q[k]) = (real_t)GSD(u, q[k]);
        }
        if (lane == 0) {
            state[0] = 1;
            state[1] = iterations;
        }
    }
    __syncthreads();
}

__device__ void gauss_seidel_wave(int N, double h2, double inv, int src, int F, double tol, int *state)
{
    if (threadIdx.x < 64) {
        const int lane = threadIdx.x;
        const int n = N * N;
        const double f = lane < n ? (double)FF(lane) : 0.0;
        int iterations = 0;
        const double u = gsw::solve<double>(N, h2, inv, f, tol, 50000000, &iterations);
        if (lane < n) SRC(lane) = (real_t)u;
        if (lane == 0) {
            state[0] = 1;
            state[1] = iterations;
        }
    }
    __syncthreads();
}

template <int CTRL>
__device__ __forceinline__ double gsp_shift(double v)
{
    return __hiloint2double(__builtin_amdgcn_update_dpp(0, __double2hiint(v), CTRL, 0xf, 0xf, true),
                            __builtin_amdgcn_update_dpp(0, __double2loint(v), CTRL, 0xf, 0xf, true));
}

__device__ __forceinline__ void gauss_seidel_blocks(int N, double h2, double inv, int src, int F, double tol, int *state)
{
    const int tid = threadIdx.x;
    if (tid < N * N) SRC(tid) = real_t(0.0);
    if (tid < 16) {
        const int lane = tid;
        const int nb = (N - 2) >> 1;
        const int br = lane >> 2, bc = lane & 3;
        const bool active = br < nb && bc < nb;
        const int r0 = 1 + 2 * br, c0 = 1 + 2 * bc;
        const int p00 = r0 * N + c0;
        double fa = 0.0, fb = 0.0, fc = 0.0, fd = 0.0;
        if (active) {
            fa = (double)FF(p00);
            fb = (double)FF(p00 + 1);
            fc = (double)FF(p00 + N);
            fd = (double)FF(p00 + N + 1);
        }
        const double q = active ? 0.25 : 0.0;
        const double qa = q * (h2 * fa), qb = q * (h2 * fb), qc = q * (h2 * fc), qd = q * (h2 * fd);
        const double keep = active ? 1.0 : 0.0;
        const double denom = (double)((N - 2) * (N - 2));
        const double thr = tol * denom, thr_hi = thr * (1.0 + 0x1p-48), thr_lo = thr * (1.0 - 0x1p-48);
        constexpr int GS_BATCH = 8;
        double fm = fmax(fmax(fabs(fa), fabs(fb)), fmax(fabs(fc), fabs(fd)));
        fm = fmax(fm, gsw::row_shr_zero<1>(fm));
        fm = fmax(fm, gsw::row_shr_zero<2>(fm));
        fm = fmax(fm, gsw::row_shr_zero<4>(fm));
        fm = fmax(fm, gsw::row_shr_zero<8>(fm));
        const double f_max = gsw::read_lane(fm, 15), k_num = thr * 0x1p31;
        int fast_until = 50000000;
        if (!(k_num >= 5e7 * f_max)) {
            const double k_safe = k_num / f_max;
            fast_until = __builtin_amdgcn_readfirstlane(k_safe > 0.0 ? (int)k_safe : 0);
        }
        const double thr_e = 0.25 * thr * h2, thr_d = 2.0 * thr_e, thr_e_hi = thr_e * (1.0 + 0x1p-10), thr_e_lo = thr_e * (1.0 - 0x1p-10);
        struct Iterate {
            double a, b, c, d;
            double a_e, d_s, d_w, a_n;
            double b_w, c_s, c_e, b_n;
        };
        auto sweep = [&](Iterate &s, double &na, double &nd) {
            s.a = na;
            s.d = nd;
            s.a_e = gsp_shift<0x101>(s.a), s.d_s = gsp_shift<0x114>(s.d), s.d_w = gsp_shift<0x111>(s.d), s.a_n = gsp_shift<0x104>(s.a);
            s.b = __builtin_fma(q, ((s.a + s.a_e) + s.d) + s.d_s, -qb);
            s.c = __builtin_fma(q, ((s.d_w + s.d) + s.a_n) + s.a, -qc);
            s.b_w = gsp_shift<0x111>(s.b);
            s.c_s = gsp_shift<0x114>(s.c);
            s.c_e = gsp_shift<0x101>(s.c);
            s.b_n = gsp_shift<0x104>(s.b);
            na = __builtin_fma(q, ((s.b_w + s.b) + s.c) + s.c_s, -qa);
            nd = __builtin_fma(q, ((s.c + s.c_e) + s.b_n) + s.b, -qd);
        };
        auto row_total = [](double acc) {
            acc += gsw::row_shr_zero<1>(acc);
            acc += gsw::row_shr_zero<2>(acc);
            acc += gsw::row_shr_zero<4>(acc);
            acc += gsw::row_shr_zero<8>(acc);
            return gsw::read_lane(acc, 15);
        };
        auto above_target = [&](const Iterate &s) {
            const double ra = inv * (s.c + s.c_s + s.b + s.b_w - 4 * s.a) - fa;
            const double rd = inv * (s.b_n + s.b + s.c_e + s.c - 4 * s.d) - fd;
            const double rb = inv * (s.d + s.d_s + s.a_e + s.a - 4 * s.b) - fb;
            const double rc = inv * (s.a_n + s.a + s.d + s.d_w - 4 * s.c) - fc;
            const double sum = row_total(keep * (fabs(ra) + fabs(rb) + fabs(rc) + fabs(rd)));
            return sum > thr_hi ? true : (sum < thr_lo ? false : sum / denom > tol);
        };
        Iterate u;
        double na = 0.0 - qa, nd = 0.0 - qd;
        int iterations = 0;
        while (iterations + GS_BATCH <= fast_until) {
            const double batch_a = na, batch_d = nd;
#pragma unroll
            for (int m = 0; m < GS_BATCH; ++m) sweep(u, na, nd);
            const double step_a = fabs(na - u.a), step_d = fabs(nd - u.d);
            bool above = __builtin_amdgcn_ballot_w64(fmax(step_a, step_d) > thr_d) != 0;
            if (!above) above = row_total(keep * (step_a + step_d)) > thr_e_hi;
            if (!above) {
                na = batch_a;
                nd = batch_d;
                break;
            }
            iterations += GS_BATCH;
        }
        for (;;) {
            sweep(u, na, nd);
            ++iterations;
            bool above, decided = false;
            if (iterations < fast_until) {
                const double est = row_total(keep * (fabs(na - u.a) + fabs(nd - u.d)));
                above = est > thr_e_hi;
                decided = above || est < thr_e_lo;
            }
            if (!decided) above = above_target(u);
            if (!above || iterations >= 50000000) break;
        }
        if (active) {
            SRC(p00) = (real_t)u.a;
            SRC(p00 + 1) = (real_t)u.b;
            SRC(p00 + N) = (real_t)u.c;
            SRC(p00 + N + 1) = (real_t)u.d;
        }
        if (lane == 0) {
            state[0] = 1;
            state[1] = iterations;
        }
    }
    __syncthreads();
}

#define ITAB(i) (reinterpret_cast<int *>(lds)[(i)])

__host__ __device__ __forceinline__ int gs_scratch(const TailArgsT<real_t> &a)
{
    size_t elems = 0;
    for (int l = 0; l < a.n_levels; ++l) elems += (size_t)3 * a.N[l] * a.N[l];
    return (int)((elems * sizeof(real_t) + 7) / 8);
}

#ifdef MG_TAIL_PHASES
#define PHASE(k) do { if (a.trace && threadIdx.x == 0 && i < 24) a.trace[TAIL_MAX_NODES + 2 + i * 8 + (k)] = clock64(); } while (0)
#else
#define PHASE(k) do { } while (0)
#endif

__device__ __forceinline__ int lane_get(int v, int l) { return __builtin_amdgcn_readlane(v, l); }
__device__ __forceinline__ float lane_get(float v, int l) { return __int_as_float(__builtin_amdgcn_readlane(__float_as_int(v), l)); }
__device__ __forceinline__ double lane_get(double v, int l)
{
    return __hiloint2double(__builtin_amdgcn_readlane(__double2hiint(v), l), __builtin_amdgcn_readlane(__double2loint(v), l));
}

__global__ __launch_bounds__(TAIL_THREADS) void k_tail(const TailArgsT<real_t> a)
{
    __shared__ double sm[17];
    __shared__ double slots[2][TAIL_WAVES];
    const real_t *a_F_top = a.F_top;
    real_t *a_U_top = a.U_top;
    double *a_err_dev = a.err_dev;
    int *a_gs_state = a.gs_state;
    if (a.batch) {
        typedef const TailBatchItem __attribute__((address_space(4))) *item_ptr;
        const item_ptr b = (item_ptr)(uintptr_t)(a.batch + blockIdx.x);
        a_F_top = static_cast<const real_t *>(b->F_top);
        a_U_top = static_cast<real_t *>(b->U_top);
        a_err_dev = b->err_dev;
        a_gs_state = b->gs_state;
    }
    const int tab_lane = threadIdx.x & 63;
    int lv_where = 0, lv_tabs = 0;
    real_t lv_dx2 = 0, lv_inv = 0, lv_cdx = 1, lv_crcp = 1;
    double lv_gs_h2 = 0, lv_gs_inv = 0;
    if (tab_lane < a.n_levels) {
        int base = 0, rt = a.tab_real0, it = a.tab_int0;
#pragma unroll
        for (int k = 0; k < TAIL_MAX_LEVELS - 1; ++k)
            if (k < tab_lane) {
                base += 3 * a.N[k] * a.N[k];
                rt += a.N[k + 1] + 4 * a.N[k];
                it += a.N[k + 1] + 2 * a.N[k];
            }
        lv_where = base | (a.N[tab_lane] << 16);
        lv_tabs = rt | (it << 16);
        lv_dx2 = a.dx2[tab_lane];
        lv_inv = a.inv[tab_lane];
        lv_gs_h2 = a.gs_h2[tab_lane];
        lv_gs_inv = a.gs_inv[tab_lane];
        if (tab_lane + 1 < a.n_levels) {
            lv_cdx = a.c_dx[tab_lane];
            lv_crcp = real_t(1.0) / lv_cdx;
        }
    }
    int nd_what = 1, nd_err = -1;
    double nd_tol = 0.0;
    if (tab_lane < a.n_nodes) {
        nd_what = (a.nodes[tab_lane].type + 1) | (a.nodes[tab_lane].steps << 2);
        nd_err = a.nodes[tab_lane].err_slot;
        nd_tol = a.nodes[tab_lane].tol;
    }
    auto N_of = [&](int l) { return lane_get(lv_where, l) >> 16; };
    auto real_tab_of = [&](int l) { return lane_get(lv_tabs, l) & 0xffff; };
    auto int_tab_of = [&](int l) { return (int)((unsigned)lane_get(lv_tabs, l) >> 16); };
    unsigned swapped = 0;
    auto U_of = [&](int l) { const int w = lane_get(lv_where, l), n = w >> 16; return (w & 0xffff) + (((swapped >> l) & 1u) ? n * n : 0); };
    auto T_of = [&](int l) { const int w = lane_get(lv_where, l), n = w >> 16; return (w & 0xffff) + (((swapped >> l) & 1u) ? 0 : n * n); };
    auto F_of = [&](int l) { const int w = lane_get(lv_where, l), n = w >> 16; return (w & 0xffff) + 2 * n * n; };
    if (a.trace && threadIdx.x == 0) a.trace[0] = wall_clock64();
    {
        const int N0 = N_of(0), f0 = F_of(0);
        for (int p = threadIdx.x; p < N0 * N0; p += TAIL_THREADS) lds[f0 + p] = a_F_top[p];
        const int wave = threadIdx.x >> 6, lane = threadIdx.x & 63;
        for (int l = 0; l + 1 < a.n_levels; ++l) {
            const int N = N_of(l), M = N_of(l + 1), rt = real_tab_of(l), it = int_tab_of(l);
            constexpr int W = TAIL_WAVES < 8 ? TAIL_WAVES : 8;
            for (int i = lane; i < N; i += 64) {
                if (wave == 0 % W && i < M) lds[rt + i] = a.r_w[l][i];
                if (wave == 1 % W) lds[rt + M + i] = a.p_rhi[l][i];
                if (wave == 2 % W) lds[rt + M + N + i] = a.p_rlo[l][i];
                if (wave == 3 % W) lds[rt + M + 2 * N + i] = a.p_chi[l][i];
                if (wave == 4 % W) lds[rt + M + 3 * N + i] = a.p_clo[l][i];
                if (wave == 5 % W && i < M) ITAB(it + i) = a.r_lo[l][i];
                if (wave == 6 % W) ITAB(it + M + i) = a.p_orow[l][i];
                if (wave == 7 % W) ITAB(it + M + N + i) = a.p_ocol[l][i];
            }
        }
    }
    __syncthreads();
    if (a.trace && threadIdx.x == 0) a.trace[1] = wall_clock64();

    int cur = 0, parity = 0;
    int pend_slot = -1, pend_N = 0, pend_parity = 0;
    auto flush_error = [&]() {
        if (pend_slot >= 0 && threadIdx.x == TAIL_THREADS - 64) finish_error(slots[pend_parity], pend_N, a_err_dev + pend_slot);
        pend_slot = -1;
    };
    const int n_nodes = a.n_nodes;
    for (int i = 0; i < n_nodes; ++i) {
        TailNode nd;
        {
            const int w = lane_get(nd_what, i);
            nd.type = (w & 3) - 1;
            nd.steps = w >> 2;
            nd.err_slot = lane_get(nd_err, i);
            nd.tol = lane_get(nd_tol, i);
        }
        if (a.trace && threadIdx.x == 0 && i > 0) a.trace[1 + i] = wall_clock64();
        flush_error();
        const int wave_first = __builtin_amdgcn_readfirstlane((int)threadIdx.x) & ~63;
        if (nd.type == -1) {
            const int N = N_of(cur);
            if (wave_first >= N * N) {
                if ((threadIdx.x & 63) == 0) slots[parity][threadIdx.x >> 6] = 0.0;
                for (int b = 0; b < nd.steps + 2; ++b) __syncthreads();
                if ((nd.steps - 1) & 1) swapped ^= 1u << cur;
                pend_slot = nd.err_slot, pend_N = N, pend_parity = parity;
                parity ^= 1;
                ++cur;
                continue;
            }
            auto down = [&](auto np_tag) {
            constexpr int NP = decltype(np_tag)::value;
            PHASE(0);
            const int F = F_of(cur);
            const PointsT<NP> P = map_points<NP>(N);
            const real_t dx2 = lane_get(lv_dx2, cur), inv = lane_get(lv_inv, cur);
            real_t v[NP], f[NP], h2f[NP];
#pragma unroll
            for (int k = 0; k < NP; ++k) {
                f[k] = P.live[k] ? lds[F + P.p[k]] : real_t(0.0);
                h2f[k] = dx2 * f[k];
                v[k] = 0.0;
            }
            PHASE(1);
            sweep<true, NP>(P, N, 0, U_of(cur), v, h2f);
            PHASE(2);
            for (int s = 1; s < nd.steps; ++s) {
                sweep<false, NP>(P, N, U_of(cur), T_of(cur), v, h2f);
                swapped ^= 1u << cur;
            }
            PHASE(3);
            const int src = U_of(cur), D = T_of(cur);
            double acc = 0.0;
#pragma unroll
            for (int k = 0; k < NP; ++k) {
                if (!P.live[k]) continue;
                const int p = P.p[k];
                real_t d = 0.0;
                if (P.inner[k]) {
                    d = inv * (SRC(p + N) + SRC(p - N) + SRC(p + 1) + SRC(p - 1) - 4 * v[k]) - f[k];
                    if (P.even[k]) acc += fabs((double)d);
                }
                lds[D + p] = -d;
            }
            post_partial(acc, slots[parity]);
            __syncthreads();
            PHASE(4);
            pend_slot = nd.err_slot, pend_N = N, pend_parity = parity;
            PHASE(5);
            parity ^= 1;
            const int M = N_of(cur + 1), Fc = F_of(cur + 1);
            const int rt = real_tab_of(cur), it = int_tab_of(cur);
            constexpr int NQ = (TAIL_MAX_N / 2) * (TAIL_MAX_N / 2) <= TAIL_THREADS ? 1 : (NP + 3) / 4;
            const PointsT<NQ> Q = map_points<NQ>(M);
#pragma unroll
            for (int k = 0; k < NQ; ++k) {
                if (!Q.live[k]) continue;
                real_t vc = 0.0;
                if (Q.inner[k]) {
                    const int rc = Q.r[k], cc = Q.c[k];
                    const real_t wa = lds[rt + cc], wb = real_t(1.0) - wa, wc = lds[rt + rc], wd = real_t(1.0) - wc;
                    const int q = D + ITAB(it + rc) * N + ITAB(it + cc);
                    const real_t u0 = lds[q], u1 = lds[q + 1], u2 = lds[q + N], u3 = lds[q + N + 1];
                    vc = wb * wd * u0 + wa * wd * u1 + wc * wb * u2 + wa * wc * u3;
                }
                lds[Fc + Q.p[k]] = vc;
            }
            };
            if (N * N <= TAIL_THREADS) down(std::integral_constant<int, 1>{});
            else if (N * N <= 2 * TAIL_THREADS) down(std::integral_constant<int, 2>{});
            else if (PT > 4 && N * N <= 4 * TAIL_THREADS) down(std::integral_constant<int, 4>{});
            else down(std::integral_constant<int, PT>{});
            __syncthreads();
            PHASE(6);
            ++cur;
        } else if (nd.type == 0) {
            const int N = N_of(cur);
            const double gs_h2 = lane_get(lv_gs_h2, cur), gs_inv = lane_get(lv_gs_inv, cur);
            if (N * N <= 64 && (N & 1) == 0 && N >= 4) {
                gauss_seidel_blocks(N, gs_h2, gs_inv, U_of(cur), F_of(cur), nd.tol, a_gs_state);
            } else if (N * N <= 64) {
                gauss_seidel_wave(N, gs_h2, gs_inv, U_of(cur), F_of(cur), nd.tol, a_gs_state);
            } else if (N * N <= 64 * GS_WAVE_PTS) {
                const bool in_place = sizeof(real_t) == sizeof(double);
                gauss_seidel_wave_lds(N, gs_h2, gs_inv, in_place ? U_of(cur) : gs_scratch(a), in_place, U_of(cur), F_of(cur),
                                      nd.tol, a_gs_state);
            } else gauss_seidel_level(N, gs_h2, gs_inv, U_of(cur), F_of(cur), gs_scratch(a), nd.tol, sm, a_gs_state);
            __syncthreads();
        } else {
            const int Nc = N_of(cur), fine = cur - 1, N = N_of(fine);
            if (wave_first >= N * N) {
                if ((threadIdx.x & 63) == 0) slots[parity][threadIdx.x >> 6] = 0.0;
                for (int b = 0; b < nd.steps + 2; ++b) __syncthreads();
                if (nd.steps & 1) swapped ^= 1u << fine;
                pend_slot = nd.err_slot, pend_N = N, pend_parity = parity;
                parity ^= 1;
                --cur;
                continue;
            }
            auto up = [&](auto np_tag) {
            constexpr int NP = decltype(np_tag)::value;
            PHASE(0);
            const int uc = U_of(cur), F = F_of(fine);
            const int rt = real_tab_of(fine) + Nc, it = int_tab_of(fine) + Nc;
            const real_t c_dx = lane_get(lv_cdx, fine), c_rcp = lane_get(lv_crcp, fine), dx2 = lane_get(lv_dx2, fine), inv = lane_get(lv_inv, fine);
            const PointsT<NP> P = map_points<NP>(N);
            real_t v[NP], f[NP], h2f[NP];
            {
                const int uf = U_of(fine);
#pragma unroll
                for (int k = 0; k < NP; ++k) {
                    f[k] = real_t(0.0);
                    v[k] = real_t(0.0);
                    if (P.live[k]) {
                        const int q = P.p[k], kf = P.r[k], l = P.c[k];
                        f[k] = lds[F + q];
                        v[k] = lds[uf + q];
                        const int ci = ITAB(it + kf), cj = ITAB(it + N + l);
                        if (ci >= 0 && cj >= 0) {
                            const int p = uc + ci * Nc + cj;
                            const real_t c1 = lds[p], c2 = lds[p + 1], c3 = lds[p + Nc], c4 = lds[p + Nc + 1];
                            const real_t rhi = lds[rt + kf], rlo = lds[rt + N + kf], chi = lds[rt + 2 * N + l], clo = lds[rt + 3 * N + l];
                            const real_t num = (c1 * chi + c2 * clo) * rhi + (c3 * chi + c4 * clo) * rlo;
                            v[k] = v[k] + div_by_const(div_by_const(num, c_dx, c_rcp), c_dx, c_rcp);
                            lds[uf + q] = v[k];
                        }
                    }
                    h2f[k] = dx2 * f[k];
                }
            }
            __syncthreads();
            PHASE(1);
            for (int s = 0; s < nd.steps; ++s) {
                sweep<false, NP>(P, N, U_of(fine), T_of(fine), v, h2f);
                swapped ^= 1u << fine;
            }
            PHASE(2);
            const int src = U_of(fine);
            double acc = 0.0;
#pragma unroll
            for (int k = 0; k < NP; ++k) {
                if (P.inner[k] && P.even[k]) {
                    const int p = P.p[k];
                    acc += fabs((double)(inv * (SRC(p + N) + SRC(p - N) + SRC(p + 1) + SRC(p - 1) - 4 * v[k]) - f[k]));
                }
            }
            post_partial(acc, slots[parity]);
            __syncthreads();
            PHASE(3);
            pend_slot = nd.err_slot, pend_N = N, pend_parity = parity;
            PHASE(4);
            };
            if (N * N <= TAIL_THREADS) up(std::integral_constant<int, 1>{});
            else if (N * N <= 2 * TAIL_THREADS) up(std::integral_constant<int, 2>{});
            else if (PT > 4 && N * N <= 4 * TAIL_THREADS) up(std::integral_constant<int, 4>{});
            else up(std::integral_constant<int, PT>{});
            parity ^= 1;
            --cur;
        }
    }
    flush_error();
    if (a.trace && threadIdx.x == 0) a.trace[1 + a.n_nodes] = wall_clock64();
    {
        const int N0 = N_of(0), u0 = U_of(0);
        for (int p = threadIdx.x; p < N0 * N0; p += TAIL_THREADS) a_U_top[p] = lds[u0 + p];
    }
}

struct TailLayout {
    int tab_real0, tab_int0;
    size_t bytes;
};
inline TailLayout tail_layout(const TailArgsT<real_t> &a)
{
    size_t bytes = 0;
    for (int l = 0; l < a.n_levels; ++l) bytes += (size_t)3 * a.N[l] * a.N[l] * sizeof(real_t);
    if (sizeof(real_t) != sizeof(double)) {
        int depth = 0, worst = 0;
        for (int i = 0; i < a.n_nodes; ++i) {
            if (a.nodes[i].type == -1) ++depth;
            else if (a.nodes[i].type == 1) --depth;
            else if (a.N[depth] * a.N[depth] > 64 && a.N[depth] > worst) worst = a.N[depth];
        }
        if (worst) bytes = (size_t)gs_scratch(a) * 8 + (size_t)2 * worst * worst * sizeof(double);
    }
    bytes = (bytes + 7) / 8 * 8;
    size_t n_real = 0, n_int = 0;
    for (int l = 0; l + 1 < a.n_levels; ++l) {
        n_real += (size_t)a.N[l + 1] + 4 * (size_t)a.N[l];
        n_int += (size_t)a.N[l + 1] + 2 * (size_t)a.N[l];
    }
    TailLayout L;
    L.tab_real0 = (int)(bytes / sizeof(real_t));
    bytes += (n_real * sizeof(real_t) + 7) / 8 * 8;
    L.tab_int0 = (int)(bytes / sizeof(int));
    bytes += n_int * sizeof(int);
    L.bytes = bytes;
    return L;
}
inline size_t tail_lds_bytes(const TailArgsT<real_t> &a) { return tail_layout(a).bytes; }

inline void tail_launch(hipStream_t s, const TailArgsT<real_t> &a, int n_batch = 1, const TailBatchItem *batch_dev = nullptr)
{
    static bool attr_set = false;
    if (!attr_set) {
        (void)hipFuncSetAttribute((const void *)k_tail, hipFuncAttributeMaxDynamicSharedMemorySize, 160 * 1024 - 512);
        attr_set = true;
    }
    const TailLayout L = tail_layout(a);
    TailArgsT<real_t> b = a;
    b.tab_real0 = L.tab_real0;
    b.tab_int0 = L.tab_int0;
    b.batch = batch_dev;
    hipLaunchKernelGGL(k_tail, dim3(batch_dev ? n_batch : 1), dim3(TAIL_THREADS), L.bytes, s, b);
}

}
}
}
```

Before: 805,200 MLUPS.

## Fold the N=128 level's pre/post smoothing into the one-workgroup tail kernel

Lets the single-workgroup tail kernel also take the 128x128 level as a register-resident top level. That level's pre-smoothing and restriction, and later its prolongation and post-smoothing, are done inside the kernel using a row-per-wave layout, DPP lane shifts and an LDS halo exchange. Lane-held level tables are stashed to LDS around the top-level work. The aim is to remove separate kernel launches and global round trips for the 128 level. The cost is more register pressure and complexity in the tail kernel, and 128^2 work runs on one CU.

```diff
diff --git a/multigrid_poisson_solver_amd/csrc/mg_cycle.cpp b/multigrid_poisson_solver_amd/csrc/mg_cycle.cpp
--- a/multigrid_poisson_solver_amd/csrc/mg_cycle.cpp
+++ b/multigrid_poisson_solver_amd/csrc/mg_cycle.cpp
@@ -201,19 +201,22 @@
 }
 
 bool scan_tail(const std::vector<double> &tokens, size_t *tok_io, const std::vector<int> &sizes, int at0, int con_step,
-               int top_N, double L, k::TailArgs *out, int *node_level)
+               int top_N, double L, k::TailArgs *out, int *node_level, bool reg_top)
 {
     static const bool disabled = getenv("MG_NO_TAIL") != nullptr;
-    if (disabled || con_step < 1 || top_N > k::TAIL_MAX_N || top_N < 3) return false;
+    if (disabled || con_step < 1 || top_N > (reg_top ? k::TAIL_MAX_TOP_N : k::TAIL_MAX_N) || top_N < 3) return false;
     k::TailArgs &a = *out;
     memset(&a, 0, sizeof a);
-    a.N[0] = top_N;
-    int depth = 0, max_depth = 0, at = at0, n_nodes = 0;
+    const int base = reg_top ? -1 : 0;
+    if (reg_top) a.top_N = top_N;
+    else a.N[0] = top_N;
+    int depth = base, max_depth = base, at = at0, n_nodes = 0;
     size_t tok = *tok_io;
     for (;;) {
+        if (reg_top && n_nodes > 0 && depth == base) break;
         if (tok >= tokens.size()) return false;
         const int node = (int)tokens[tok++];
-        if (node == 1 && depth == 0) {
+        if (node == 1 && depth == base) {
             --tok;
             break;
         }
@@ -225,20 +228,22 @@
         if (node == -1) {
             if (at + 1 >= (int)sizes.size() || depth + 1 >= k::TAIL_MAX_LEVELS) return false;
             nd.steps = con_step;
+            nd.top = depth < 0 ? 1 : 0;
             node_level[n_nodes] = depth;
             ++depth;
             a.N[depth] = sizes[(size_t)++at];
-            if (a.N[depth] < 3) return false;
+            if (a.N[depth] < 3 || (depth == 0 && reg_top && a.N[0] * 2 != top_N)) return false;
             if (depth > max_depth) max_depth = depth;
         } else if (node == 0) {
             if (tok + 1 >= tokens.size()) return false;
             nd.tol = tokens[tok++];
-            if ((int)tokens[tok++] != 1) return false;
+            if ((int)tokens[tok++] != 1 || depth < 0) return false;
             node_level[n_nodes] = depth;
         } else if (node == 1) {
             nd.steps = con_step;
             --depth;
             --at;
+            nd.top = depth < 0 ? 1 : 0;
             node_level[n_nodes] = depth;
         } else {
             return false;
@@ -248,6 +253,25 @@
     if (n_nodes == 0 || at != at0) return false;
     a.n_nodes = n_nodes;
     a.n_levels = max_depth + 1;
+    if (reg_top) {
+        if (a.n_levels < 1 || a.nodes[0].type != -1) return false;
+        const RestrictTable &rt = restrict_table(top_N, a.N[0]);
+        const ProlongTable &pt = prolong_table(a.N[0], top_N);
+        if (!rt.lo || !rt.fusable || !pt.owner_row || !pt.fusable) return false;
+        const double dx = L / (double)(top_N - 1);
+        a.top_dx2 = dx * dx;
+        a.top_inv = 1.0 / a.top_dx2;
+        a.top_r_inv = rt.inv;
+        a.top_r_wf = rt.inv_w;
+        a.top_p_orow = pt.owner_row;
+        a.top_p_ocol = pt.owner_col;
+        a.top_p_rhi = pt.row_hi;
+        a.top_p_rlo = pt.row_lo;
+        a.top_p_chi = pt.col_hi;
+        a.top_p_clo = pt.col_lo;
+        a.top_c_dx = pt.c_dx;
+        a.top_c_rcp = 1.0 / a.top_c_dx;
+    }
     if (!k::tail_fits(a)) return false;
     for (int l = 0; l < a.n_levels; ++l) {
         const double dx = L / (double)(a.N[l] - 1);
@@ -419,11 +443,18 @@
     LevelNode *top = cycle.last();
     static const int batch_tail_n = [] { const char *e = getenv("MG_BATCH_TAIL_N"); return e ? atoi(e) : 32; }();
     if (x.tracing && top->N > batch_tail_n) return false;
+    static const int tail_top_n = [] { const char *e = getenv("MG_TAIL_TOP_N"); return e ? atoi(e) : k::TAIL_MAX_N; }();
+    const bool reg_top = top->N > k::TAIL_MAX_N;
+    if (reg_top && (top->N > tail_top_n || top->N > k::TAIL_MAX_TOP_N || (top->N & 1) || (p->flags & MG_CYCLE_MIXED) || x.tracing ||
+                    x.c.smoother != SMOOTHER_STREAM || !k::stream_fusable(top->N) || p->con_step > k::tile_max_steps()))
+        return false;
+    const bool restart = reg_top && cycle.Get_init() == 0 && cycle.Is_firstNode();
 
     k::TailArgs a;
     int node_level[k::TAIL_MAX_NODES];
     size_t tok = x.tok;
-    if (!scan_tail(p->tokens, &tok, p->sizes, x.at, p->con_step, top->N, p->L, &a, node_level)) return false;
+    if (!scan_tail(p->tokens, &tok, p->sizes, x.at, p->con_step, top->N, p->L, &a, node_level, reg_top)) return false;
+    if (restart) a.nodes[0].top = 2;
     const int n_nodes = a.n_nodes;
     if (p->records.size() + (size_t)n_nodes > p->err_cap) return false;
     const int rec0 = (int)p->records.size();
@@ -431,7 +462,7 @@
     const char *up = "             *\n             |\nProlongation |\n             |\n             *\n";
     for (int i = 0; i < n_nodes; ++i) {
         k::TailNode &nd = a.nodes[i];
-        const int N = a.N[node_level[i]];
+        const int N = node_level[i] < 0 ? a.top_N : a.N[node_level[i]];
         if (nd.type == -1) {
             const int rec = add_record(p, -1, N, nd.steps);
             nd.err_slot = rec - rec0;
@@ -500,14 +531,14 @@
         ++traced;
         fprintf(stderr, "[tail trace] staging %.2f us;", (double)(t[1] - t[0]) * 0.01);
         for (int i = 0; i < a.n_nodes; ++i)
-            fprintf(stderr, " %d@%d:%.2f", a.nodes[i].type, a.N[node_level[i]], (double)(t[(size_t)i + 2] - t[(size_t)i + 1]) * 0.01);
+            fprintf(stderr, " %d@%d:%.2f", a.nodes[i].type, node_level[i] < 0 ? a.top_N : a.N[node_level[i]], (double)(t[(size_t)i + 2] - t[(size_t)i + 1]) * 0.01);
         fprintf(stderr, " us\n");
 #ifdef MG_TAIL_PHASES
         std::vector<long long> ph(24 * 8);
         (void)hipMemcpy(ph.data(), trace + k::TAIL_MAX_NODES + 2, ph.size() * sizeof(long long), hipMemcpyDeviceToHost);
         for (int i = 0; i < a.n_nodes && i < 24; ++i) {
             if (a.nodes[i].type == 0) continue;
-            fprintf(stderr, "[tail phases] %2d@%-3d cycles:", a.nodes[i].type, a.N[node_level[i]]);
+            fprintf(stderr, "[tail phases] %2d@%-3d cycles:", a.nodes[i].type, node_level[i] < 0 ? a.top_N : a.N[node_level[i]]);
             for (int k = 1; k < 8 && ph[(size_t)i * 8 + k]; ++k) fprintf(stderr, " %lld", ph[(size_t)i * 8 + k] - ph[(size_t)i * 8 + k - 1]);
             fprintf(stderr, "\n");
         }
@@ -515,6 +546,11 @@
         (void)hipFree(trace);
     }
     x.tok = tok;
+    if (reg_top) {
+        top->pending_pre = 0;
+        top->descents++;
+        if (cycle.Is_firstNode()) cycle.Set_init(0);
+    }
     return true;
 }
 
@@ -547,6 +583,12 @@
         if (x.c.last_error) { x.status = 10; break; }
         if (p->records.size() >= p->err_cap) { x.status = 11; break; }
 
+        if (node == -1 && fused && !mixed && !x.tracing && cycle.Is_firstNode() && cycle.last()->N > k::TAIL_MAX_N &&
+            cycle.last()->N <= k::TAIL_MAX_TOP_N) {
+            --x.tok;
+            if (try_tail(x)) continue;
+            ++x.tok;
+        }
         if (node == -1) {
             int step = 0, next_N = 0;
             if (p->con_step == 0) { if (!x.next_int(&step)) { x.status = 3; break; } }
@@ -780,7 +822,7 @@
     if (a.kind != b.kind || a.node.N != b.node.N) return false;
     if (a.kind == 2) {
         const k::TailArgs &x = p->tails[(size_t)a.tail], &y = p->tails[(size_t)b.tail];
-        if (x.n_levels != y.n_levels || x.n_nodes != y.n_nodes) return false;
+        if (x.n_levels != y.n_levels || x.n_nodes != y.n_nodes || x.top_N != y.top_N) return false;
         for (int l = 0; l < x.n_levels; ++l)
             if (x.N[l] != y.N[l]) return false;
         for (int i = 0; i < x.n_nodes; ++i) {
diff --git a/multigrid_poisson_solver_amd/csrc/mg_internal.h b/multigrid_poisson_solver_amd/csrc/mg_internal.h
--- a/multigrid_poisson_solver_amd/csrc/mg_internal.h
+++ b/multigrid_poisson_solver_amd/csrc/mg_internal.h
@@ -292,11 +292,12 @@
 constexpr int TAIL_MAX_LEVELS = 6;
 constexpr int TAIL_MAX_NODES = 48;
 constexpr int TAIL_MAX_N = 64;
+constexpr int TAIL_MAX_TOP_N = 128;
 struct TailNode {
     int type;
     int steps;
     int err_slot;
-    int pad;
+    int top;
     double tol;
 };
 template <typename T>
@@ -317,6 +318,12 @@
     double *err_dev;
     int *gs_state;
     const TailBatchItem *batch;
+    int top_N, top_stash;
+    T top_dx2, top_inv, top_c_dx, top_c_rcp;
+    const int *top_r_inv;
+    const T *top_r_wf;
+    const int *top_p_orow, *top_p_ocol;
+    const T *top_p_rhi, *top_p_rlo, *top_p_chi, *top_p_clo;
     TailNode nodes[TAIL_MAX_NODES];
 };
 typedef TailArgsT<double> TailArgs;
@@ -535,6 +542,6 @@
                              int step, double *error_dev);
 k::TailArgsF tail_args_f32(const k::TailArgs &a);
 bool scan_tail(const std::vector<double> &tokens, size_t *tok_io, const std::vector<int> &sizes, int at0, int con_step,
-               int top_N, double L, k::TailArgs *out, int *node_level);
+               int top_N, double L, k::TailArgs *out, int *node_level, bool reg_top = false);
 
 }
diff --git a/multigrid_poisson_solver_amd/csrc/mg_tail.hip b/multigrid_poisson_solver_amd/csrc/mg_tail.hip
--- a/multigrid_poisson_solver_amd/csrc/mg_tail.hip
+++ b/multigrid_poisson_solver_amd/csrc/mg_tail.hip
@@ -10,7 +10,7 @@
     const int n = N * N, t = threadIdx.x;
     if (t < n) f64::lds[n + t] = F[t];
     __syncthreads();
-    f64::gauss_seidel_blocks(N, h2, inv, 0, n, tol, state);
+    f64::gauss_seidel_blocks(N, h2, inv, 0, n, tol, state, t);
     if (t < n) U[t] = f64::lds[t];
 }
 void gauss_seidel_blocks_launch(hipStream_t s, int N, double h2, double inv, double *U, const double *F, double tol, int *state)
diff --git a/multigrid_poisson_solver_amd/csrc/mg_tail_impl.h b/multigrid_poisson_solver_amd/csrc/mg_tail_impl.h
--- a/multigrid_poisson_solver_amd/csrc/mg_tail_impl.h
+++ b/multigrid_poisson_solver_amd/csrc/mg_tail_impl.h
@@ -5,6 +5,7 @@
 #include "mg_divconst.h"
 #include "mg_gs_wave.h"
 #include "mg_internal.h"
+#include "mg_lane_ops.h"
 
 #if !defined(MG_REAL) || !defined(MG_REAL_NS)
 #error "define MG_REAL (double|float) and MG_REAL_NS (f64|f32) before including mg_tail_impl.h"
@@ -63,13 +64,13 @@
     bool live[NP], inner[NP], even[NP];
 };
 template <int NP>
-__device__ __forceinline__ PointsT<NP> map_points(int N)
+__device__ __forceinline__ PointsT<NP> map_points(int N, int tid)
 {
     PointsT<NP> P;
     const float rn = 1.0f / (float)N;
 #pragma unroll
     for (int k = 0; k < NP; ++k) {
-        const int p = (int)threadIdx.x + k * TAIL_THREADS;
+        const int p = tid + k * TAIL_THREADS;
         const int r = (int)(((float)p + 0.5f) * rn), c = p - r * N;
         P.p[k] = p;
         P.r[k] = r;
@@ -167,10 +168,10 @@
 }
 
 constexpr int GS_WAVE_PTS = 4;
-__device__ void gauss_seidel_wave_lds(int N, double h2, double inv, int u, bool in_place, int src, int F, double tol, int *state)
-{
-    if (threadIdx.x < 64) {
-        const int lane = threadIdx.x, n = N * N;
+__device__ void gauss_seidel_wave_lds(int N, double h2, double inv, int u, bool in_place, int src, int F, double tol, int *state, int tid)
+{
+    if (tid < 64) {
+        const int lane = tid, n = N * N;
         const float rn = 1.0f / (float)N;
         int q[GS_WAVE_PTS];
         bool live[GS_WAVE_PTS], inner[GS_WAVE_PTS], red[GS_WAVE_PTS];
@@ -240,10 +241,10 @@
     __syncthreads();
 }
 
-__device__ void gauss_seidel_wave(int N, double h2, double inv, int src, int F, double tol, int *state)
-{
-    if (threadIdx.x < 64) {
-        const int lane = threadIdx.x;
+__device__ void gauss_seidel_wave(int N, double h2, double inv, int src, int F, double tol, int *state, int tid)
+{
+    if (tid < 64) {
+        const int lane = tid;
         const int n = N * N;
         const double f = lane < n ? (double)FF(lane) : 0.0;
         int iterations = 0;
@@ -264,9 +265,8 @@
                             __builtin_amdgcn_update_dpp(0, __double2loint(v), CTRL, 0xf, 0xf, true));
 }
 
-__device__ __forceinline__ void gauss_seidel_blocks(int N, double h2, double inv, int src, int F, double tol, int *state)
-{
-    const int tid = threadIdx.x;
+__device__ __forceinline__ void gauss_seidel_blocks(int N, double h2, double inv, int src, int F, double tol, int *state, int tid)
+{
     if (tid < N * N) SRC(tid) = real_t(0.0);
     if (tid < 16) {
         const int lane = tid;
@@ -398,6 +398,243 @@
     return __hiloint2double(__builtin_amdgcn_readlane(__double2hiint(v), l), __builtin_amdgcn_readlane(__double2loint(v), l));
 }
 
+constexpr int TOP_RPW = (TAIL_MAX_TOP_N + TAIL_WAVES - 1) / TAIL_WAVES;
+constexpr int TOP_STRIDE = TAIL_MAX_TOP_N;
+constexpr int TOP_XCH_REALS = 2 * TAIL_WAVES * 2 * TOP_STRIDE;
+
+struct TopLane {
+    int N, wave, x0, yb;
+    real_t q0, q1;
+    int xb;
+};
+__device__ __forceinline__ TopLane top_lane(int N, int tid)
+{
+    TopLane t;
+    t.N = N;
+    t.wave = __builtin_amdgcn_readfirstlane(tid >> 6);
+    t.x0 = 2 * (tid & 63);
+    t.yb = t.wave * TOP_RPW;
+    t.q0 = (t.x0 <= 0 || t.x0 >= N - 1) ? real_t(0.0) : real_t(0.25);
+    t.q1 = (t.x0 + 1 >= N - 1) ? real_t(0.0) : real_t(0.25);
+    t.xb = 0;
+    return t;
+}
+__device__ __forceinline__ int top_row_inner(const TopLane &t, int j) { return ((unsigned)(t.yb + j - 1) < (unsigned)(t.N - 2)) ? -1 : 0; }
+__device__ __forceinline__ const real_t *top_row(const TopLane &t, const real_t *A, int j)
+{
+    const int y = t.yb + j;
+    return A + (unsigned)((y < t.N ? y : t.N - 1) * t.N);
+}
+__device__ __forceinline__ unsigned top_col(const TopLane &t) { return (unsigned)(t.x0 < t.N ? t.x0 : t.N - 2); }
+__device__ __forceinline__ int top_live(const TopLane &t, int j) { return (t.yb + j < t.N && t.x0 < t.N) ? -1 : 0; }
+
+__device__ __forceinline__ void top_exchange(TopLane &t, const real_t (&first)[2], const real_t (&last)[2], real_t (&below)[2], real_t (&above)[2])
+{
+    const int mine = ((t.xb * TAIL_WAVES + t.wave) * 2) * TOP_STRIDE + t.x0;
+    lds[mine] = first[0];
+    lds[mine + 1] = first[1];
+    lds[mine + TOP_STRIDE] = last[0];
+    lds[mine + TOP_STRIDE + 1] = last[1];
+    __syncthreads();
+    below[0] = below[1] = above[0] = above[1] = real_t(0.0);
+    if (t.wave > 0) {
+        below[0] = lds[mine - TOP_STRIDE];
+        below[1] = lds[mine - TOP_STRIDE + 1];
+    }
+    if (t.wave < TAIL_WAVES - 1) {
+        above[0] = lds[mine + 2 * TOP_STRIDE];
+        above[1] = lds[mine + 2 * TOP_STRIDE + 1];
+    }
+    t.xb ^= 1;
+}
+
+__device__ __forceinline__ void top_sweep(TopLane &t, real_t (&v)[TOP_RPW][2], const real_t (&f)[TOP_RPW][2], real_t dx2)
+{
+    asm volatile("" : "+s"(dx2));
+    real_t q0 = t.q0, q1 = t.q1;
+    asm volatile("" : "+v"(q0), "+v"(q1));
+    real_t so[2], above[2];
+    top_exchange(t, v[0], v[TOP_RPW - 1], so, above);
+#pragma unroll
+    for (int j = 0; j < TOP_RPW; ++j) {
+        const real_t c0 = v[j][0], c1 = v[j][1];
+        const real_t n0 = j < TOP_RPW - 1 ? v[j < TOP_RPW - 1 ? j + 1 : 0][0] : above[0];
+        const real_t n1 = j < TOP_RPW - 1 ? v[j < TOP_RPW - 1 ? j + 1 : 0][1] : above[1];
+        const real_t w0 = from_lane_below(c1), e1 = from_lane_above(c0);
+        const int inner = top_row_inner(t, j);
+        const real_t t0 = minus4(n0 + so[0] + c1 + w0, c0) - dx2 * f[j][0];
+        const real_t t1 = minus4(n1 + so[1] + e1 + c0, c1) - dx2 * f[j][1];
+        v[j][0] = fused_mul_add(hi_bits_and(q0, inner), t0, c0);
+        v[j][1] = fused_mul_add(hi_bits_and(q1, inner), t1, c1);
+        so[0] = c0;
+        so[1] = c1;
+    }
+}
+__device__ __forceinline__ void top_sweep_zero(const TopLane &t, real_t (&v)[TOP_RPW][2], const real_t (&f)[TOP_RPW][2], real_t dx2)
+{
+#pragma unroll
+    for (int j = 0; j < TOP_RPW; ++j) {
+        const int inner = top_row_inner(t, j);
+        v[j][0] = fused_mul_add(hi_bits_and(t.q0, inner), real_t(0.0) - dx2 * f[j][0], real_t(0.0));
+        v[j][1] = fused_mul_add(hi_bits_and(t.q1, inner), real_t(0.0) - dx2 * f[j][1], real_t(0.0));
+    }
+}
+template <bool SIGNED>
+__device__ __forceinline__ double top_residual(TopLane &t, const real_t (&v)[TOP_RPW][2], real_t (&f)[TOP_RPW][2], real_t inv)
+{
+    real_t so[2], above[2];
+    top_exchange(t, v[0], v[TOP_RPW - 1], so, above);
+    double acc = 0.0;
+    const real_t ms0 = t.q0 == real_t(0.0) ? real_t(0.0) : real_t(-1.0), ms1 = t.q1 == real_t(0.0) ? real_t(0.0) : real_t(-1.0);
+    const int even0 = (t.yb & 1) == 0 ? -1 : 0;
+#pragma unroll
+    for (int j = 0; j < TOP_RPW; ++j) {
+        const real_t c0 = v[j][0], c1 = v[j][1];
+        const real_t n0 = j < TOP_RPW - 1 ? v[j < TOP_RPW - 1 ? j + 1 : 0][0] : above[0];
+        const real_t n1 = j < TOP_RPW - 1 ? v[j < TOP_RPW - 1 ? j + 1 : 0][1] : above[1];
+        const real_t w0 = from_lane_below(c1), e1 = from_lane_above(c0);
+        const int inner = top_row_inner(t, j);
+        const real_t r0 = inv * minus4(n0 + so[0] + c1 + w0, c0) - f[j][0];
+        const real_t r1 = inv * minus4(n1 + so[1] + e1 + c0, c1) - f[j][1];
+        const int row_even = (j & 1) ? ~even0 : even0;
+        const int m0 = (t.q0 == real_t(0.0) ? 0 : inner) & row_even, m1 = (t.q1 == real_t(0.0) ? 0 : inner) & ~row_even;
+        acc += fabs(bits_and((double)r0, m0));
+        acc += fabs(bits_and((double)r1, m1));
+        if (SIGNED) {
+            f[j][0] = r0 * hi_bits_and(ms0, inner);
+            f[j][1] = r1 * hi_bits_and(ms1, inner);
+        }
+        so[0] = c0;
+        so[1] = c1;
+    }
+    return acc;
+}
+__device__ __forceinline__ void top_store(const TopLane &t, const real_t (&v)[TOP_RPW][2], real_t *U)
+{
+#pragma unroll
+    for (int j = 0; j < TOP_RPW; ++j)
+        if (top_live(t, j)) {
+            real_t *row = const_cast<real_t *>(top_row(t, U, j)) + top_col(t);
+            row[0] = v[j][0];
+            row[1] = v[j][1];
+        }
+}
+__device__ __forceinline__ void top_load(const TopLane &t, const real_t *A, real_t (&v)[TOP_RPW][2])
+{
+#pragma unroll
+    for (int j = 0; j < TOP_RPW; ++j) {
+        const real_t *row = top_row(t, A, j) + top_col(t);
+        v[j][0] = bits_and(row[0], top_live(t, j));
+        v[j][1] = bits_and(row[1], top_live(t, j));
+    }
+}
+
+template <typename Args>
+__device__ __forceinline__ double top_down(Args a, const real_t *F_top, real_t *U_top, bool from_U, int steps, int Fc, int M, int tid)
+{
+    TopLane t = top_lane(a->top_N, tid);
+    const int lane = tid & 63;
+    real_t v[TOP_RPW][2], f[TOP_RPW][2];
+    top_load(t, F_top, f);
+    if (from_U) top_load(t, U_top, v);
+    const real_t dx2 = a->top_dx2, inv = a->top_inv;
+    int s = 0;
+    if (!from_U) {
+        top_sweep_zero(t, v, f, dx2);
+        s = 1;
+    }
+    for (; s < steps; ++s) top_sweep(t, v, f, dx2);
+    __builtin_amdgcn_sched_barrier(0);
+    const int yl = t.yb + (lane < TOP_RPW ? lane : TOP_RPW - 1), ylc = yl < t.N ? yl : t.N - 1;
+    const int xc = t.x0 < t.N ? t.x0 : t.N - 2;
+    const int t_rc = (yl < t.N && lane < TOP_RPW) ? a->top_r_inv[ylc] : -1;
+    const real_t t_rw = a->top_r_wf[ylc];
+    const int rc0 = a->top_r_inv[xc], rc1 = a->top_r_inv[xc + 1];
+    const real_t rwf0 = a->top_r_wf[xc], rwf1 = a->top_r_wf[xc + 1];
+    const bool second = rc1 >= 0;
+    const int rc_col = t.x0 < t.N ? (second ? rc1 : rc0) : -1;
+    const real_t rw_a = second ? rwf1 : rwf0;
+    top_store(t, v, U_top);
+    const double acc = top_residual<true>(t, v, f, inv);
+    real_t unused[2], d_next[2];
+    top_exchange(t, f[0], f[TOP_RPW - 1], unused, d_next);
+    (void)unused;
+    __syncthreads();
+    const real_t rw_b = real_t(1.0) - rw_a;
+#pragma unroll
+    for (int j = 0; j < TOP_RPW; ++j) {
+        const int rc_row = lane_value(t_rc, j);
+        const real_t a0 = f[j][0], a1 = f[j][1];
+        const real_t b0 = j < TOP_RPW - 1 ? f[j < TOP_RPW - 1 ? j + 1 : 0][0] : d_next[0];
+        const real_t b1 = j < TOP_RPW - 1 ? f[j < TOP_RPW - 1 ? j + 1 : 0][1] : d_next[1];
+        const real_t a2 = from_lane_above(a0), b2 = from_lane_above(b0);
+        if (rc_row < 0) continue;
+        const real_t wc = lane_value(t_rw, j), wd = real_t(1.0) - wc;
+        const real_t u0 = second ? a1 : a0, u1 = second ? a2 : a1, u2 = second ? b1 : b0, u3 = second ? b2 : b1;
+        const real_t vc = rw_b * wd * u0 + rw_a * wd * u1 + wc * rw_b * u2 + rw_a * wc * u3;
+        if (rc_col >= 0) lds[Fc + rc_row * M + rc_col] = vc;
+    }
+    if (tid < M) {
+        const int i = tid;
+        lds[Fc + i] = real_t(0.0);
+        lds[Fc + (M - 1) * M + i] = real_t(0.0);
+        lds[Fc + i * M] = real_t(0.0);
+        lds[Fc + i * M + M - 1] = real_t(0.0);
+    }
+    return acc;
+}
+
+template <typename Args>
+__device__ __forceinline__ double top_up(Args a, const real_t *F_top, real_t *U_top, int steps, int uc, int Nc, int tid)
+{
+    TopLane t = top_lane(a->top_N, tid);
+    const int lane = tid & 63;
+    real_t v[TOP_RPW][2], f[TOP_RPW][2], pv[TOP_RPW][2];
+    const int yl = t.yb + (lane < TOP_RPW ? lane : TOP_RPW - 1), ylc = yl < t.N ? yl : t.N - 1;
+    const int xc = t.x0 < t.N ? t.x0 : t.N - 2;
+    const int t_own = a->top_p_orow[ylc];
+    const real_t t_rhi = a->top_p_rhi[ylc], t_rlo = a->top_p_rlo[ylc];
+    const int cj[2] = {a->top_p_ocol[xc], a->top_p_ocol[xc + 1]};
+    const real_t chi[2] = {a->top_p_chi[xc], a->top_p_chi[xc + 1]}, clo[2] = {a->top_p_clo[xc], a->top_p_clo[xc + 1]};
+    const real_t c_dx = a->top_c_dx, c_rcp = a->top_c_rcp, dx2 = a->top_dx2, inv = a->top_inv;
+    {
+        real_t hA[2] = {0, 0}, hB[2] = {0, 0};
+        int c_row = -2;
+#pragma unroll
+        for (int j = 0; j < TOP_RPW; ++j) {
+            const int own = lane_value(t_own, j);
+            if (own != c_row) {
+                const bool step_one = own == c_row + 1;
+#pragma unroll
+                for (int c = 0; c < 2; ++c) {
+                    const int p = uc + own * Nc + cj[c];
+                    hA[c] = step_one ? hB[c] : lds[p] * chi[c] + lds[p + 1] * clo[c];
+                    hB[c] = lds[p + Nc] * chi[c] + lds[p + Nc + 1] * clo[c];
+                }
+                c_row = own;
+            }
+            const real_t own_yh = lane_value(t_rhi, j), own_yl = lane_value(t_rlo, j);
+#pragma unroll
+            for (int c = 0; c < 2; ++c) {
+                const real_t num = hA[c] * own_yh + hB[c] * own_yl;
+                pv[j][c] = div_by_const(div_by_const(num, c_dx, c_rcp), c_dx, c_rcp);
+            }
+        }
+    }
+    __builtin_amdgcn_sched_barrier(0);
+    top_load(t, U_top, v);
+    top_load(t, F_top, f);
+#pragma unroll
+    for (int j = 0; j < TOP_RPW; ++j) {
+        v[j][0] = v[j][0] + bits_and(pv[j][0], top_live(t, j));
+        v[j][1] = v[j][1] + bits_and(pv[j][1], top_live(t, j));
+    }
+    __syncthreads();
+    for (int s = 0; s < steps; ++s) top_sweep(t, v, f, dx2);
+    top_store(t, v, U_top);
+    return top_residual<false>(t, v, f, inv);
+}
+
 __global__ __launch_bounds__(TAIL_THREADS) void k_tail(const TailArgsT<real_t> a)
 {
     __shared__ double sm[17];
@@ -438,11 +675,12 @@
             lv_crcp = real_t(1.0) / lv_cdx;
         }
     }
-    int nd_what = 1, nd_err = -1;
+    int nd_what = 1, nd_err = -1, nd_top = 0;
     double nd_tol = 0.0;
     if (tab_lane < a.n_nodes) {
         nd_what = (a.nodes[tab_lane].type + 1) | (a.nodes[tab_lane].steps << 2);
         nd_err = a.nodes[tab_lane].err_slot;
+        nd_top = a.nodes[tab_lane].top;
         nd_tol = a.nodes[tab_lane].tol;
     }
     auto N_of = [&](int l) { return lane_get(lv_where, l) >> 16; };
@@ -452,10 +690,12 @@
     auto U_of = [&](int l) { const int w = lane_get(lv_where, l), n = w >> 16; return (w & 0xffff) + (((swapped >> l) & 1u) ? n * n : 0); };
     auto T_of = [&](int l) { const int w = lane_get(lv_where, l), n = w >> 16; return (w & 0xffff) + (((swapped >> l) & 1u) ? 0 : n * n); };
     auto F_of = [&](int l) { const int w = lane_get(lv_where, l), n = w >> 16; return (w & 0xffff) + 2 * n * n; };
+    const bool has_top = sizeof(real_t) == sizeof(double) && a.top_N != 0;
     if (a.trace && threadIdx.x == 0) a.trace[0] = wall_clock64();
     {
         const int N0 = N_of(0), f0 = F_of(0);
-        for (int p = threadIdx.x; p < N0 * N0; p += TAIL_THREADS) lds[f0 + p] = a_F_top[p];
+        if (!has_top)
+            for (int p = threadIdx.x; p < N0 * N0; p += TAIL_THREADS) lds[f0 + p] = a_F_top[p];
         const int wave = threadIdx.x >> 6, lane = threadIdx.x & 63;
         for (int l = 0; l + 1 < a.n_levels; ++l) {
             const int N = N_of(l), M = N_of(l + 1), rt = real_tab_of(l), it = int_tab_of(l);
@@ -475,7 +715,7 @@
     __syncthreads();
     if (a.trace && threadIdx.x == 0) a.trace[1] = wall_clock64();
 
-    int cur = 0, parity = 0;
+    int cur = has_top ? -1 : 0, parity = 0;
     int pend_slot = -1, pend_N = 0, pend_parity = 0;
     auto flush_error = [&]() {
         if (pend_slot >= 0 && threadIdx.x == TAIL_THREADS - 64) finish_error(slots[pend_parity], pend_N, a_err_dev + pend_slot);
@@ -483,6 +723,8 @@
     };
     const int n_nodes = a.n_nodes;
     for (int i = 0; i < n_nodes; ++i) {
+        int tid = threadIdx.x;
+        asm volatile("" : "+v"(tid));
         TailNode nd;
         {
             const int w = lane_get(nd_what, i);
@@ -494,6 +736,39 @@
         if (a.trace && threadIdx.x == 0 && i > 0) a.trace[1 + i] = wall_clock64();
         flush_error();
         const int wave_first = __builtin_amdgcn_readfirstlane((int)threadIdx.x) & ~63;
+        if (has_top && nd.type != 0 && cur == (nd.type == -1 ? -1 : 0)) {
+            typedef const TailArgsT<real_t> __attribute__((address_space(4))) *args_ptr;
+            args_ptr ap = (args_ptr)__builtin_amdgcn_kernarg_segment_ptr();
+            asm volatile("" : "+s"(ap));
+            const int st = ap->top_stash;
+            if (wave_first == 0) {
+                const int vals[19] = {lv_where, lv_tabs, __double2hiint(lv_dx2), __double2loint(lv_dx2), __double2hiint(lv_inv), __double2loint(lv_inv),
+                                      __double2hiint(lv_cdx), __double2loint(lv_cdx), __double2hiint(lv_crcp), __double2loint(lv_crcp),
+                                      __double2hiint(lv_gs_h2), __double2loint(lv_gs_h2), __double2hiint(lv_gs_inv), __double2loint(lv_gs_inv),
+                                      nd_what, nd_err, nd_top, __double2hiint(nd_tol), __double2loint(nd_tol)};
+#pragma unroll
+                for (int k = 0; k < 19; ++k) ITAB(st + 64 * k + tab_lane) = vals[k];
+            }
+            double acc;
+            if (nd.type == -1) acc = top_down(ap, a_F_top, a_U_top, lane_get(nd_top, i) == 2, nd.steps, F_of(0), N_of(0), tid);
+            else acc = top_up(ap, a_F_top, a_U_top, nd.steps, U_of(0), N_of(0), tid);
+            post_partial(acc, slots[parity]);
+            __syncthreads();
+            {
+                int vals[19];
+#pragma unroll
+                for (int k = 0; k < 19; ++k) vals[k] = ITAB(st + 64 * k + tab_lane);
+                lv_where = vals[0], lv_tabs = vals[1];
+                lv_dx2 = (real_t)__hiloint2double(vals[2], vals[3]), lv_inv = (real_t)__hiloint2double(vals[4], vals[5]);
+                lv_cdx = (real_t)__hiloint2double(vals[6], vals[7]), lv_crcp = (real_t)__hiloint2double(vals[8], vals[9]);
+                lv_gs_h2 = __hiloint2double(vals[10], vals[11]), lv_gs_inv = __hiloint2double(vals[12], vals[13]);
+                nd_what = vals[14], nd_err = vals[15], nd_top = vals[16], nd_tol = __hiloint2double(vals[17], vals[18]);
+            }
+            pend_slot = nd.err_slot, pend_N = ap->top_N, pend_parity = parity;
+            parity ^= 1;
+            cur = nd.type == -1 ? 0 : -1;
+            continue;
+        }
         if (nd.type == -1) {
             const int N = N_of(cur);
             if (wave_first >= N * N) {
@@ -509,7 +784,7 @@
             constexpr int NP = decltype(np_tag)::value;
             PHASE(0);
             const int F = F_of(cur);
-            const PointsT<NP> P = map_points<NP>(N);
+            const PointsT<NP> P = map_points<NP>(N, tid);
             const real_t dx2 = lane_get(lv_dx2, cur), inv = lane_get(lv_inv, cur);
             real_t v[NP], f[NP], h2f[NP];
 #pragma unroll
@@ -548,7 +823,7 @@
             const int M = N_of(cur + 1), Fc = F_of(cur + 1);
             const int rt = real_tab_of(cur), it = int_tab_of(cur);
             constexpr int NQ = (TAIL_MAX_N / 2) * (TAIL_MAX_N / 2) <= TAIL_THREADS ? 1 : (NP + 3) / 4;
-            const PointsT<NQ> Q = map_points<NQ>(M);
+            const PointsT<NQ> Q = map_points<NQ>(M, tid);
 #pragma unroll
             for (int k = 0; k < NQ; ++k) {
                 if (!Q.live[k]) continue;
@@ -574,13 +849,13 @@
             const int N = N_of(cur);
             const double gs_h2 = lane_get(lv_gs_h2, cur), gs_inv = lane_get(lv_gs_inv, cur);
             if (N * N <= 64 && (N & 1) == 0 && N >= 4) {
-                gauss_seidel_blocks(N, gs_h2, gs_inv, U_of(cur), F_of(cur), nd.tol, a_gs_state);
+                gauss_seidel_blocks(N, gs_h2, gs_inv, U_of(cur), F_of(cur), nd.tol, a_gs_state, tid);
             } else if (N * N <= 64) {
-                gauss_seidel_wave(N, gs_h2, gs_inv, U_of(cur), F_of(cur), nd.tol, a_gs_state);
+                gauss_seidel_wave(N, gs_h2, gs_inv, U_of(cur), F_of(cur), nd.tol, a_gs_state, tid);
             } else if (N * N <= 64 * GS_WAVE_PTS) {
                 const bool in_place = sizeof(real_t) == sizeof(double);
                 gauss_seidel_wave_lds(N, gs_h2, gs_inv, in_place ? U_of(cur) : gs_scratch(a), in_place, U_of(cur), F_of(cur),
-                                      nd.tol, a_gs_state);
+                                      nd.tol, a_gs_state, tid);
             } else gauss_seidel_level(N, gs_h2, gs_inv, U_of(cur), F_of(cur), gs_scratch(a), nd.tol, sm, a_gs_state);
             __syncthreads();
         } else {
@@ -600,7 +875,7 @@
             const int uc = U_of(cur), F = F_of(fine);
             const int rt = real_tab_of(fine) + Nc, it = int_tab_of(fine) + Nc;
             const real_t c_dx = lane_get(lv_cdx, fine), c_rcp = lane_get(lv_crcp, fine), dx2 = lane_get(lv_dx2, fine), inv = lane_get(lv_inv, fine);
-            const PointsT<NP> P = map_points<NP>(N);
+            const PointsT<NP> P = map_points<NP>(N, tid);
             real_t v[NP], f[NP], h2f[NP];
             {
                 const int uf = U_of(fine);
@@ -659,18 +934,20 @@
     if (a.trace && threadIdx.x == 0) a.trace[1 + a.n_nodes] = wall_clock64();
     {
         const int N0 = N_of(0), u0 = U_of(0);
-        for (int p = threadIdx.x; p < N0 * N0; p += TAIL_THREADS) a_U_top[p] = lds[u0 + p];
+        if (!has_top)
+            for (int p = threadIdx.x; p < N0 * N0; p += TAIL_THREADS) a_U_top[p] = lds[u0 + p];
     }
 }
 
 struct TailLayout {
-    int tab_real0, tab_int0;
+    int tab_real0, tab_int0, top_stash;
     size_t bytes;
 };
 inline TailLayout tail_layout(const TailArgsT<real_t> &a)
 {
     size_t bytes = 0;
     for (int l = 0; l < a.n_levels; ++l) bytes += (size_t)3 * a.N[l] * a.N[l] * sizeof(real_t);
+    if (a.top_N && bytes < (size_t)TOP_XCH_REALS * sizeof(real_t)) bytes = (size_t)TOP_XCH_REALS * sizeof(real_t);
     if (sizeof(real_t) != sizeof(double)) {
         int depth = 0, worst = 0;
         for (int i = 0; i < a.n_nodes; ++i) {
@@ -691,6 +968,8 @@
     bytes += (n_real * sizeof(real_t) + 7) / 8 * 8;
     L.tab_int0 = (int)(bytes / sizeof(int));
     bytes += n_int * sizeof(int);
+    L.top_stash = (int)(bytes / sizeof(int));
+    if (a.top_N) bytes += 19 * 64 * sizeof(int);
     L.bytes = bytes;
     return L;
 }
@@ -707,6 +986,7 @@
     TailArgsT<real_t> b = a;
     b.tab_real0 = L.tab_real0;
     b.tab_int0 = L.tab_int0;
+    b.top_stash = L.top_stash;
     b.batch = batch_dev;
     hipLaunchKernelGGL(k_tail, dim3(batch_dev ? n_batch : 1), dim3(TAIL_THREADS), L.bytes, s, b);
 }
```

Result: no change. 805,200 MLUPS (-0.0%).
